# jeong0982/gkr

Measured on AMD Instinct MI355X. Metric: BN254-Fr sumcheck field-ops/sec @ 2^20 vars, higher is better.
Workload: dtype u32x8

## Files before the change

### gkr_amd/csrc/capi_internal.h

```cpp
#pragma once
#include <hip/hip_runtime.h>
#include <sched.h>
#include <stdio.h>
#include <stdlib.h>
#include <string.h>

#include <algorithm>
#include <chrono>
#include <condition_variable>
#include <map>
#include <memory>
#include <mutex>
#include <string>
#include <thread>
#include <vector>

#include "../../include/gkr_amd.h"
#include "fr64.h"
#include "host_cpus.h"
#include "hostpool.h"
#include "kernels.h"
#include "options.h"
#include "gate_seg.h"
#include "keccak.h"
// ... 63 lines not shown
    static const bool adx = !gkr::process_switch("GKR_NO_ADX") && gkr::gkr_adx_available();
    if (!adx) return gkr::h64::mimc7_multi_hash(arr, n, cts, nullptr);
    gkr::h64::F out;
    gkr::gkr_adx_multi_hash(reinterpret_cast<const uint64_t(*)[4]>(arr), n, reinterpret_cast<const uint64_t(*)[4]>(cts), out.l);
    return out;
}

constexpr int kHashChunkMax = 16;
constexpr int kMaxLayerK = GKR_MAX_K_NEXT, kMaxLayerKi = GKR_MAX_K_I, kMaxDenseK = GKR_MAX_K_NEXT_DEVICE_TRANSCRIPT;
inline void ifma_hash_chunk(const uint64_t (*vec)[3][4], const uint32_t* ln, int count, uint64_t (*out)[4]) {
    if (count > 8)
        gkr::gkr_ifma_multi_hash16(vec, ln, 3, out);
    else
        gkr::gkr_ifma_multi_hash8(vec, ln, 3, out);
}
inline int hash_chunk_size(int tables, int threads, int help_share = 0) {
    const long long forced = gkr::opt(gkr::OPT_hash_chunk);
    if (forced == 8 || forced == 16) return (int)forced;
    if (help_share > 1 && tables <= 3 * help_share) return 1;
    return tables >= 32 * threads ? 16 : 8;
}

inline hipError_t device_malloc(void** p, size_t bytes) { return hipMalloc(p, bytes); }
inline hipError_t device_free(void* p) { return hipFree(p); }

inline int default_host_threads() {
    if (const int v = gkr::process_int("GKR_HOST_THREADS", 0); v >= 1) return v;
    int cpus = usable_cpus();
    int local = 1;
    if (const int ranks = gkr::process_int("LOCAL_WORLD_SIZE", 1); ranks > 0) local = ranks;
    const int share = cpus / local;
    int t = share >= 6 ? share - 2 : (share >= 3 ? share - 1 : share);
    if (t < 1) t = 1;
    if (t > 64) t = 64;
    return t;
}

inline Fr to_dev(const gkr_fr& x) {
    Fr f;
    memcpy(&f, &x, 32);
    return f;
}

inline gkr_fr to_abi(const Fr& x) {
    gkr_fr f;
    memcpy(&f, &x, 32);
    return f;
}

inline bool all_canonical(const gkr_fr* v, size_t n) {
    for (size_t i = 0; i < n; ++i)
        if (!gkr::fr_is_canonical(to_dev(v[i]))) return false;
    return true;
}


}
using namespace gkr_host;


struct GateLists {
    uint32_t *offsets = nullptr, *cursor = nullptr, *list = nullptr;
    uint32_t* plan = nullptr;
    gkr::GatePlanCounts plan_counts{};
    gkr::GateSegs segs;
    bool ready = false;
    void release() {
        if (offsets) (void)hipFree(offsets);
        if (cursor) (void)hipFree(cursor);
        if (list) (void)hipFree(list);
        if (plan) (void)hipFree(plan);
        if (segs.words) (void)hipFree(segs.words);
        offsets = cursor = list = plan = nullptr;
        plan_counts = gkr::GatePlanCounts{};
        segs = gkr::GateSegs();
        ready = false;
    }
};
struct PreparedCircuit {
    uint64_t h1 = 0, h2 = 0;
    std::vector<uint32_t> k;
    std::vector<uint8_t*> gt;
    std::vector<uint32_t*> l, r;
    std::vector<GateLists> lists;
    std::vector<unsigned char> retained;
    void release() {
        for (auto p : gt) (void)hipFree(p);
        for (auto p : l) (void)hipFree(p);
        for (auto p : r) (void)hipFree(p);
        for (auto& g : lists) g.release();
        gt.clear();
        l.clear();
        r.clear();
        lists.clear();
    }
};

struct ProveCrew;

struct AsyncWorker {
    std::thread th;
    std::mutex mu;
    std::condition_variable cv;
    std::function<void()> task;
    bool busy = false, stop = false;
    void loop() {
        std::unique_lock<std::mutex> g(mu);
        for (;;) {
            cv.wait(g, [this] { return stop || (busy && task); });
            if (stop) return;
            std::function<void()> t = std::move(task);
            task = nullptr;
            g.unlock();
            t();
            g.lock();
            busy = false;
            cv.notify_all();
        }
    }
    void run(std::function<void()> fn) {
        std::unique_lock<std::mutex> g(mu);
        if (!th.joinable()) th = std::thread([this] { loop(); });
        cv.wait(g, [this] { return !busy; });
        task = std::move(fn);
        busy = true;
        cv.notify_all();
    }
    void wait() {
        std::unique_lock<std::mutex> g(mu);
        cv.wait(g, [this] { return !busy; });
    }
    ~AsyncWorker() {
        {
            std::unique_lock<std::mutex> g(mu);
            cv.wait(g, [this] { return !busy; });
            stop = true;
            cv.notify_all();
        }
        if (th.joinable()) th.join();
    }
};

struct gkr_ctx {
    int device = 0;
    std::vector<int> devices;
    int host_threads = 0;
    gkr::Options options = gkr::Options::from_environment();
    std::vector<std::unique_ptr<PreparedCircuit>> circuits;
    hipStream_t stream = nullptr;
    hipStream_t aux = nullptr;
    hipStream_t late = nullptr;
    hipStream_t chain = nullptr;
    std::vector<hipEvent_t> aux_events;
    Fr* d_cts = nullptr;
    int transcript = GKR_TRANSCRIPT_HOST;
    std::string err;
    int profile = 0;
    std::map<std::string, ProfileRow> prof;
    std::vector<PendingEvent> pending;
    std::vector<hipEvent_t> event_pool;
    char name[256] = {0};
    uint32_t ticket = 0;
    std::unique_ptr<gkr::SpinPool> pool;
    std::unique_ptr<gkr::SpinPool> solo_pool;
    std::unique_ptr<AsyncWorker> copier;
    std::unique_ptr<AsyncWorker> liner;
    void* mle_arrivals_zeroed = nullptr;
    void* arrivals_zeroed = nullptr;
    void* gate_arrive_zeroed = nullptr;
    bool crew_member = false;
    int help_share = 0;
    int rounds_ahead = 0;
    std::unique_ptr<ProveCrew, void (*)(ProveCrew*)> crew{nullptr, nullptr};
    std::map<std::string, std::pair<void*, size_t>> ws;
    std::map<std::string, std::pair<void*, size_t>> pinned;

    hipError_t workspace(const char* slot, size_t bytes, void** out) {
        auto& e = ws[slot];
        if (e.second < bytes) {
            if (e.first) (void)device_free(e.first);
            e.first = nullptr;
            e.second = 0;
            hipError_t rc = device_malloc(&e.first, bytes);
            if (rc != hipSuccess) return rc;
            e.second = bytes;
        }
        *out = e.first;
        return hipSuccess;
    }
    hipError_t pinned_host(const char* slot, size_t bytes, void** out) {
        auto& e = pinned[slot];
        if (e.second < bytes) {
            if (e.first) (void)hipHostFree(e.first);
            e.first = nullptr;
            e.second = 0;
            hipError_t rc = hipHostMalloc(&e.first, bytes, hipHostMallocCoherent | hipHostMallocMapped);
            if (rc != hipSuccess) return rc;
            memset(e.first, 0, bytes);
            e.second = bytes;
        }
        *out = e.first;
        return hipSuccess;
    }
    void release_buffers() {
        for (auto& c : circuits) c->release();
        circuits.clear();
        for (auto& kv : ws)
            if (kv.second.first) (void)device_free(kv.second.first);
        ws.clear();
        for (auto& kv : pinned)
            if (kv.second.first) (void)hipHostFree(kv.second.first);
        pinned.clear();
    }
    int threads() const { return host_threads > 0 ? host_threads : default_host_threads(); }
    gkr::SpinPool* host_pool() {
        if (crew_member) {
            if (!solo_pool) solo_pool.reset(new gkr::SpinPool(0));
            return solo_pool.get();
        }
        if (!pool) pool.reset(new gkr::SpinPool(threads() - 1));
        return pool.get();
    }
    hipError_t late_stream(hipStream_t* out) {
        if (!late) {
            const hipError_t rc = hipStreamCreateWithFlags(&late, hipStreamNonBlocking);
            if (rc != hipSuccess) return rc;
        }
        *out = late;
        return hipSuccess;
    }
    hipError_t chain_stream(hipStream_t* out) {
        if (!chain) {
            hipError_t rc = hipStreamCreateWithFlags(&chain, hipStreamNonBlocking);
            if (rc != hipSuccess) return rc;
        }
        *out = chain;
        return hipSuccess;
    }
    hipError_t aux_stream(int events) {
        if (!aux) {
            hipError_t rc = hipStreamCreateWithFlags(&aux, hipStreamNonBlocking);
            if (rc != hipSuccess) return rc;
        }
        while ((int)aux_events.size() < events) {
            hipEvent_t e;
            hipError_t rc = hipEventCreateWithFlags(&e, hipEventDisableTiming);
            if (rc != hipSuccess) return rc;
            aux_events.push_back(e);
        }
        return hipSuccess;
    }

    int fail(int status, const std::string& what) {
        err = what;
        return status;
    }
    int hip_fail(hipError_t e, const char* what) {
        err = std::string(what) + ": " + hipGetErrorString(e);
        return GKR_ERR_HIP;
    }
    hipEvent_t get_event() {
        if (!event_pool.empty()) {
            hipEvent_t e = event_pool.back();
            event_pool.pop_back();
            return e;
        }
        hipEvent_t e;
        (void)hipEventCreate(&e);
        return e;
    }
    void add_host_sample(const char* name, double ms) {
        ProfileRow& r = prof[name];
        r.launches += 1;
        r.total_ms += ms;
        if (r.samples.size() < kMaxSamples) r.samples.emplace_back((float)ms, 0.0);
    }
    void drain_events() {
        for (auto& p : pending) {
            (void)hipEventSynchronize(p.stop);
            float ms = 0.f;
            (void)hipEventElapsedTime(&ms, p.start, p.stop);
            ProfileRow& r = prof[p.name];
            r.launches += 1;
            r.total_ms += ms;
            r.bytes += p.bytes;
            if (r.samples.size() < kMaxSamples) r.samples.emplace_back(ms, p.bytes);
            event_pool.push_back(p.start);
            event_pool.push_back(p.stop);
        }
        pending.clear();
    }
};

struct ProveCrew {
    struct Member {
        gkr_ctx* ctx = nullptr;
        std::thread th;
        std::vector<int> items;
    };
    std::vector<std::unique_ptr<Member>> members;
    std::mutex mu;
    std::condition_variable cv_start, cv_done;
    uint64_t generation = 0;
    bool stop = false;
    int active = 0;
    int finished = 0;
    gkr_prove_item* items = nullptr;
    const std::vector<std::vector<int>>* units = nullptr;
    int32_t busy = 0;
    double t_call_us = 0;
};

struct Timed {
    gkr_ctx* c;
    PendingEvent ev;
    bool on;
    hipStream_t st;
    Timed(gkr_ctx* ctx, const char* name, double bytes, hipStream_t stream = nullptr, bool minor = false)
        : c(ctx), on(ctx->profile == 1 || (ctx->profile == 2 && !minor)), st(stream ? stream : ctx->stream) {
        if (on) {
            ev.start = c->get_event();
            ev.stop = c->get_event();
            ev.name = name;
            ev.bytes = bytes;
            (void)hipEventRecord(ev.start, st);
        }
    }
    ~Timed() {
        if (on) {
            (void)hipEventRecord(ev.stop, st);
            c->pending.push_back(ev);
        }
    }
};

#define GKR_ENTER(ctx)                                        \
    HIP_TRY(ctx, hipSetDevice((ctx)->device));                \
    gkr::OptionScope gkr_option_scope_(&(ctx)->options)

#define HIP_TRY(ctx, expr)                                   \
    do {                                                     \
        hipError_t _e = (expr);                              \
        if (_e != hipSuccess) return (ctx)->hip_fail(_e, #expr); \
    } while (0)


namespace gkr_host {


template <typename T>
struct DevBuf {
    T* p = nullptr;
    ~DevBuf() {
        if (p) (void)hipFree(p);
    }
    hipError_t alloc(size_t count) { return hipMalloc(reinterpret_cast<void**>(&p), count * sizeof(T)); }
};

template <typename Run>
int run_on_upload(gkr_ctx* ctx, const gkr_fr* host, size_t count, Run run) {
    GKR_ENTER(ctx);
    DevBuf<Fr> d;
    HIP_TRY(ctx, d.alloc(count));
    HIP_TRY(ctx, hipMemcpyAsync(d.p, host, count * sizeof(Fr), hipMemcpyHostToDevice, ctx->stream));
    return run(d.p);
}
template <typename Run>
int run_on_tables(gkr_ctx* ctx, const gkr_fr* tables, size_t count, Run run) {
    if (!all_canonical(tables, count)) return ctx->fail(GKR_ERR_NON_CANONICAL, "table entry >= r");
    return run_on_upload(ctx, tables, count, run);
}

struct ThreadTimeAccount {
    double own_pieces_us = 0, helped_us = 0, spin_us = 0;
};
inline thread_local ThreadTimeAccount t_account;
struct HostAccountTotals {
    std::atomic<uint64_t> own_ns{0}, helped_ns{0}, spin_ns{0}, rest_ns{0}, lent_ns{0}, lent_idle_ns{0}, calls{0}, wake_ns{0};
    std::atomic<uint64_t> pieces{0}, piece_ns{0}, piece_pass_ns{0}, lanes[17] = {};
    std::atomic<bool> on{false};
};
inline HostAccountTotals& host_account_totals() {
    static HostAccountTotals t;
    return t;
}
inline bool accounting_on() { return host_account_totals().on.load(std::memory_order_relaxed); }
inline void account_piece(int transcripts, double pass_us, double total_us) {
    HostAccountTotals& t = host_account_totals();
    t.pieces.fetch_add(1, std::memory_order_relaxed);
    t.piece_ns.fetch_add((uint64_t)(total_us * 1e3), std::memory_order_relaxed);
    t.piece_pass_ns.fetch_add((uint64_t)(pass_us * 1e3), std::memory_order_relaxed);
    t.lanes[transcripts < 1 ? 1 : (transcripts > 16 ? 16 : transcripts)].fetch_add(1, std::memory_order_relaxed);
}
inline double now_us_dbg() { return std::chrono::duration<double, std::micro>(std::chrono::steady_clock::now().time_since_epoch()).count(); }

inline bool help_enabled() {
    static const bool on = !gkr::process_switch("GKR_NO_HELP");
    return on;
}
static void run_pieces(gkr::SpinPool* pool, const std::function<bool()>* work, bool several, int priority = 0) {
    auto run = [&] {
        if (pool)
            pool->run_now(work);
        else
            while ((*work)()) {
// ... 216 lines not shown
```

### gkr_amd/csrc/capi_mle_passes.hip

```cpp
#include "capi_internal.h"

namespace gkr_host {

void host_pass_scalar(const uint64_t* sums, size_t sums_row_words, int count, int J, const uint32_t* final_len,
                             uint64_t (*c0)[16][4], uint64_t (*c1)[16][4], uint64_t (*r)[16][4], uint32_t (*len)[16],
                             uint64_t* weights, size_t w_row_words) {
    using gkr::h64::F;
    const F* cts = host_mimc_constants64();
    const F one_m = gkr::h64::to_mont(F{{1, 0, 0, 0}});
    for (int k = 0; k < count; ++k) {
        F S[gkr::kMleMaxSub], rm[gkr::kMlePassMaxRounds];
        memcpy(S, sums + (size_t)k * sums_row_words, sizeof(F) << J);
        for (int t = 0; t < J; ++t) {
            const int half = 1 << (J - t - 1);
            F lo = S[0], hi = S[half];
            for (int b = 1; b < half; ++b) {
                lo = gkr::h64::add(lo, S[b]);
                hi = gkr::h64::add(hi, S[half + b]);
            }
            const F d = gkr::h64::sub(hi, lo);
            const uint32_t ln = (final_len && t == J - 1) ? final_len[k] : (gkr::h64::is_zero(d) ? 1u : 2u);
            const F vec[2] = {d, lo};
            const F rc = host_multi_hash(vec + (2 - ln), (int)ln, cts);
            memcpy(c0[t][k], &lo, 32);
            memcpy(c1[t][k], &d, 32);
            memcpy(r[t][k], &rc, 32);
            len[t][k] = ln;
            rm[t] = gkr::h64::to_mont(rc);
            for (int b = 0; b < half; ++b) S[b] = gkr::h64::add(S[b], gkr::h64::mont_mul(gkr::h64::sub(S[half + b], S[b]), rm[t]));
        }
        if (!weights) continue;
        F* w = reinterpret_cast<F*>(weights + (size_t)k * w_row_words);
        F tmp[gkr::kMleMaxSub];
        tmp[0] = one_m;
        int cur = 1;
        for (int t = 0; t < J; ++t) {
            const F nr = gkr::h64::sub(one_m, rm[t]);
            for (int b = cur; b-- > 0;) {
                tmp[2 * b + 1] = gkr::h64::mont_mul(tmp[b], rm[t]);
                tmp[2 * b] = gkr::h64::mont_mul(tmp[b], nr);
            }
            cur <<= 1;
        }
        memcpy(w, tmp, sizeof(F) << J);
    }
}

struct MlePassTables {
    const Fr* input = nullptr;
    size_t in_stride = 0;
    Fr* work = nullptr;
    size_t work_len = 0;
    gkr::MleSubPartial* partials = nullptr;
    unsigned char* plans = nullptr;
    Fr* h_w = nullptr;
    Fr *h_w2 = nullptr, *d_w2 = nullptr;
    gkr::MleHostRecSub* h_rec = nullptr;
    gkr::MleHostRecSub* rec = nullptr;
    uint32_t* arrivals = nullptr;
    Fr* h_tail = nullptr;
};
static int mle_pass_tables(gkr_ctx* ctx, const std::string& prefix, const Fr* input, size_t len, size_t work_len, int batch, MlePassTables& T) {
    T.input = input;
    T.in_stride = len;
    T.work_len = work_len;
    WS(ctx, (prefix + ".work").c_str(), Fr, (size_t)batch * (work_len ? work_len : 1), T.work);
    WS(ctx, (prefix + ".partials").c_str(), gkr::MleSubPartial, (size_t)batch * gkr::kMaxBlocksPerTable, T.partials);
    WS(ctx, (prefix + ".plans").c_str(), unsigned char, (size_t)batch * gkr::mle_fold_plan_bytes(), T.plans);
    HIP_TRY(ctx, ctx->pinned_host((prefix + ".rec").c_str(), sizeof(gkr::MleHostRecSub) * batch, reinterpret_cast<void**>(&T.h_rec)));
    HIP_TRY(ctx, ctx->pinned_host((prefix + ".w").c_str(), sizeof(Fr) * gkr::kMleMaxSub * batch, reinterpret_cast<void**>(&T.h_w)));
    T.rec = T.h_rec;
    return GKR_OK;
}

constexpr double kFusedPublishBytes = 64.0 * 1024 * 1024;
constexpr uint32_t kFusedPublishBlocks = 256;
constexpr size_t kArrivalCounters = 4096;
static int mle_arrival_counters(gkr_ctx* ctx, size_t len, MlePassTables& T) {
    if (gkr::opt(gkr::OPT_no_fused_reduce) != 0 || (double)len * 32.0 > kFusedPublishBytes) return GKR_OK;
    WS(ctx, "mlep.arrivals", uint32_t, kArrivalCounters, T.arrivals);
    if (ctx->mle_arrivals_zeroed != T.arrivals) {
        HIP_TRY(ctx, hipMemsetAsync(T.arrivals, 0, sizeof(uint32_t) * kArrivalCounters, ctx->stream));
        ctx->mle_arrivals_zeroed = T.arrivals;
    }
    return GKR_OK;
}
static bool fused_publish(const MlePassTables& T, int b0, int nb, uint32_t nblk, double bytes_read, uint32_t ticket, int jout, gkr::MlePublish& pub) {
    if (!T.arrivals || (size_t)(b0 + nb) > kArrivalCounters || bytes_read > kFusedPublishBytes || (uint64_t)nblk * nb > kFusedPublishBlocks || nblk > 128u)
        return false;
    pub.rec = T.rec + b0;
    pub.arrivals = T.arrivals + b0;
    pub.ticket = ticket;
    pub.jout = (uint32_t)jout;
    return true;
}

constexpr uint32_t kMleTailLog2 = 7;
struct MlePassPolicy {
    const char* row = nullptr;
    int plan_event = -1;
    Fr* export_tail = nullptr;
    int blocks_jout = 0;
    uint32_t src_planes = 1;
};
static uint32_t pass0_blocks(size_t len, int jout, int nb, const MlePassPolicy& P) {
    uint32_t nblk = gkr::mle_pass_blocks((uint32_t)len, (uint32_t)(P.blocks_jout > 0 ? P.blocks_jout : jout), nb);
    if (P.blocks_jout > 0 && len / nblk < 256u) nblk = (uint32_t)(len / 256u);
    return nblk;
}
static void queue_sub_reduce(gkr_ctx* ctx, const MlePassTables& T, int b0, int nb, uint32_t nblk, int jout, uint32_t ticket, hipStream_t st) {
    Timed t(ctx, "mle_sub_reduce", 0.0, st, true);
    gkr::launch_mle_sub_reduce(T.partials + (size_t)b0 * gkr::kMaxBlocksPerTable, nblk, (uint32_t)jout, nb, T.rec + b0, ticket, st);
}
static void queue_pass0(gkr_ctx* ctx, const MlePassTables& T, int b0, int nb, int jout, uint32_t ticket, hipStream_t st, const MlePassPolicy& P) {
    const size_t len = T.in_stride;
    const Fr* src = T.input + (size_t)b0 * len;
    const double bytes = (double)nb * len * 32.0;
    if (len <= gkr::kSmallPassEntries) {
        Timed t(ctx, "mle_pass_small", bytes, st, true);
        gkr::launch_mle_multifold_small(0, src, len, nullptr, 0, (uint32_t)len, (uint32_t)jout, nb, T.h_w + (size_t)b0 * gkr::kMleMaxSub, T.rec + b0, ticket, st);
        return;
    }
    const uint32_t nblk = pass0_blocks(len, jout, nb, P);
    gkr::MlePublish pub;
    const bool fused = fused_publish(T, b0, nb, nblk, bytes, ticket, jout, pub);
    {
        Timed t(ctx, P.row, bytes, st, fused);
        gkr::launch_mle_sub_sums(src, len, (uint32_t)len, nb, nblk, T.partials + (size_t)b0 * gkr::kMaxBlocksPerTable, st, fused ? &pub : nullptr);
    }
    if (!fused) queue_sub_reduce(ctx, T, b0, nb, nblk, jout, ticket, st);
}
static void queue_fold(gkr_ctx* ctx, const MlePassTables& T, int b0, int nb, bool from_input, int m_src, int jin, int jout, uint32_t ticket,
                       hipStream_t st, const MlePassPolicy& P) {
    const size_t src_len = (size_t)1 << m_src, S = src_len >> jin;
    const Fr* src = from_input ? T.input + (size_t)b0 * T.in_stride : T.work + (size_t)b0 * T.work_len;
    const size_t src_stride = from_input ? T.in_stride : T.work_len;
    Fr* dst = T.work + (size_t)b0 * T.work_len;
    const Fr* w = T.h_w + (size_t)b0 * gkr::kMleMaxSub;
    const double bytes = (double)nb * ((double)src_len * P.src_planes + (double)S) * 32.0;
    if (S <= gkr::kSmallPassEntries) {
        Timed t(ctx, "mle_pass_small", bytes, st, true);
        gkr::launch_mle_multifold_small(jin, src, src_stride, dst, T.work_len, (uint32_t)S, (uint32_t)jout, nb, w, T.rec + b0, ticket, st, P.export_tail,
                                        1u << kMleTailLog2, P.src_planes, (uint32_t)src_len);
        return;
    }
    const uint32_t nblk = gkr::mle_multifold_blocks((uint32_t)S, (uint32_t)jout, nb);
    unsigned char* plan = T.plans + (size_t)b0 * gkr::mle_fold_plan_bytes();
    if (gkr::mle_multifold_uses_mfma((uint32_t)S, nblk)) {
        if (P.plan_event < 0) {
            gkr::launch_mle_fold_plan(jin, w, plan, nb, st);
        } else {
            {
                Timed t(ctx, "mle_fold_plan", 0.0, ctx->aux, true);
                gkr::launch_mle_fold_plan(jin, w, plan, nb, ctx->aux);
            }
            (void)hipEventRecord(ctx->aux_events[P.plan_event], ctx->aux);
            (void)hipStreamWaitEvent(st, ctx->aux_events[P.plan_event], 0);
        }
    }
    gkr::MlePublish pub;
    const bool fused = fused_publish(T, b0, nb, nblk, (double)nb * (double)src_len * 32.0, ticket, jout, pub);
    {
        Timed t(ctx, P.row, bytes, st, fused);
        gkr::launch_mle_multifold(jin, src, src_stride, dst, T.work_len, (uint32_t)S, nb, nblk, w, plan, T.partials + (size_t)b0 * gkr::kMaxBlocksPerTable, st,
                                  fused ? &pub : nullptr);
    }
    if (!fused) queue_sub_reduce(ctx, T, b0, nb, nblk, jout, ticket, st);
}

struct MleSchedule {
    int jmax = 0, j_first = 0;
    int n_dev = 0;
    int groups = 0, depth = 0;
    int bound[kMaxGroups + 1];
    uint32_t chunk[kMaxGroups];
    bool tail_on = false;
    bool two_level = false;
};
static MleSchedule mle_schedule(int n, int batch, int hash_threads, bool is_tail, const gkr::Options& o) {
    MleSchedule sc;
    const double len = (double)((size_t)1 << n);
    const int jcap = o.v[gkr::OPT_no_mfma_fold] ? 3 : gkr::kMlePassMaxRounds;
    const int jwant = o.v[gkr::OPT_rounds_per_pass] > 0 ? (int)o.v[gkr::OPT_rounds_per_pass] : jcap;
    sc.jmax = jwant > jcap ? jcap : jwant;
    sc.j_first = mle_pass_rounds(n, n, sc.jmax);
    sc.two_level = !is_tail && mle_two_level_first_fold(n, o);
    const long long dp = o.v[gkr::OPT_device_hash_percent];
    const int dev_percent = dp < 0 ? 0 : (dp > 90 ? 90 : (int)dp);
    if (dev_percent > 0 && !is_tail && batch >= 64 && sc.j_first >= 1) {
        sc.n_dev = (int)((long long)batch * dev_percent / 100) & ~7;
        if (batch - sc.n_dev < 16) sc.n_dev = (batch - 16) & ~7;
        if (sc.n_dev < 8) sc.n_dev = 0;
    }
    const int host_batch = batch - sc.n_dev;
    const double batch_bytes = (double)host_batch * len * 32.0;
    int want_groups = (int)(batch_bytes / (4.0 * 1024 * 1024 * 1024));
    want_groups = want_groups < 4 ? 4 : (want_groups > 8 ? (batch_bytes > 96.0 * 1024 * 1024 * 1024 ? 16 : 8) : want_groups);
    const bool small_tables = n <= 17 && host_batch >= 256;
    if (small_tables) want_groups = 16;
    if (hash_threads <= 3 && host_batch >= 256 && want_groups < 16) want_groups = 16;
    int group_size = host_batch >= 128 ? (host_batch + want_groups - 1) / want_groups : (host_batch >= 16 ? (host_batch + 1) / 2 : host_batch);
    if (sc.n_dev && hash_threads <= 3 && host_batch >= 256) group_size = 64;
    if (o.v[gkr::OPT_group_size] > 0) group_size = (int)o.v[gkr::OPT_group_size];
    sc.groups = (host_batch + group_size - 1) / group_size;
    if (sc.groups > kMaxGroups) sc.groups = kMaxGroups;
    const long long forced = o.v[gkr::OPT_hash_chunk];
    for (int g = 0; g <= sc.groups; ++g) sc.bound[g] = sc.n_dev + (int)((long long)host_batch * g / sc.groups);
    for (int g = 0; g < sc.groups; ++g) {
        const int nb = sc.bound[g + 1] - sc.bound[g], per = (nb + hash_threads - 1) / hash_threads;
        sc.chunk[g] = forced == 8 || forced == 16 ? (uint32_t)forced : (nb >= 32 * hash_threads ? 16u : (uint32_t)(per <= 8 ? 8 : (per <= 16 ? per : 16)));
    }
    sc.depth = o.v[gkr::OPT_pass_queue_depth] > 0 ? (int)o.v[gkr::OPT_pass_queue_depth] : (small_tables ? 4 : 2);
    sc.tail_on = o.v[gkr::OPT_host_tail_log2] >= 0 && sc.n_dev == 0 && batch <= (o.v[gkr::OPT_host_tail_max_batch] > 0 ? o.v[gkr::OPT_host_tail_max_batch] : 8);
    return sc;
}

namespace {
struct PassGroup : GroupHandoff {
    int m = 0;
    int j = 0;
    int round0 = 0;
    int pass = 0, index = 0;
    hipStream_t chain = nullptr;
    bool on_host = false;
    bool mid = false, planes = false;
};
struct MlePassClock {
    const bool on = gkr::debug_timing();
    const std::chrono::steady_clock::time_point t0 = std::chrono::steady_clock::now();
    double a = 0, b = 0, c = 0, d = 0, e = 0;
    std::atomic<uint64_t> busy_ns{0};
    double us() const { return std::chrono::duration<double, std::micro>(std::chrono::steady_clock::now() - t0).count(); }
    void report(int threads) const {
        if (!on) return;
        fprintf(stderr,
                "[gkr timing] setup %.0f us, first launches %.0f, loop %.0f, end_session %.0f, sync %.0f, drain %.0f; hashing %.0f us "
                "over %d threads = %.0f%% of the loop\n",
                a, b - a, c - b, d - c, e - d, us() - e, busy_ns.load() * 1e-3, threads, busy_ns.load() * 1e-3 / ((c - b) * threads) * 100.0);
    }
};

struct MlePassRun {
    gkr_ctx* ctx;
    const int n, batch;
    const MleTailArgs* tail;
    gkr_fr* out_coeffs;
    uint32_t* out_len;
    gkr_fr* out_r;
    MleSchedule sc;
    MlePassTables T;
    hipStream_t s = nullptr, late = nullptr, chain = nullptr;
    std::vector<PassGroup> grp;
    std::vector<uint32_t> dep_last;
    int next_first = 0;
    gkr_fr *stage_c = nullptr, *stage_r = nullptr;
    uint32_t* stage_len = nullptr;
    MlePassClock clock;

    int rounds_for(int m) const { return mle_pass_rounds(m, n, sc.jmax); }
    void advance(PassGroup& G, int jin) {
        G.m -= jin;
        G.round0 += jin;
        G.j = rounds_for(G.m);
        G.ticket = ++ctx->ticket;
    }
    void launch_first(PassGroup& G) {
        G.ticket = ++ctx->ticket;
        MlePassPolicy P;
        P.row = G.chain ? "mle_sub_sums_dev" : "mle_sub_sums";
        if (two_level(G)) P.blocks_jout = kMleTwoLevelRounds;
        queue_pass0(ctx, T, G.b0, G.nb, G.j, G.ticket, G.chain ? G.chain : s, P);
    }
    void launch_next_first() {
        if (next_first < sc.groups) launch_first(grp[next_first++]);
    }
    void launch_fold(PassGroup& G, int jin) {
        const int m_src = G.m;
        const bool from_input = m_src == n;
        hipStream_t st = G.chain ? G.chain : ((!from_input && m_src <= 16) ? late : s);
        advance(G, jin);
        MlePassPolicy P;
        P.row = G.chain ? "mle_multifold_dev" : (st == s ? "mle_multifold" : "mle_multifold_late");
        if (!gkr::opt(gkr::OPT_plan_main) && st == s && sc.groups != 1) P.plan_event = G.index;
        G.on_host = sc.tail_on && !G.chain && G.m <= (int)kMleTailLog2 && G.m - G.j > 0;
        if (G.on_host) P.export_tail = T.h_tail + ((size_t)G.b0 << kMleTailLog2);
        if (G.planes) P.src_planes = gkr::kMleFold2Planes;
        G.planes = false;
        queue_fold(ctx, T, G.b0, G.nb, from_input, m_src, jin, G.j, G.ticket, st, P);
    }
    bool two_level(const PassGroup& G) const { return sc.two_level && !G.chain; }
    bool side_launches() const { return !gkr::opt(gkr::OPT_plan_main) && sc.groups != 1; }
    void launch_fine_sums(PassGroup& G) {
        const int J = G.j;
        G.mid = true;
        G.round0 += J;
        G.ticket = ++ctx->ticket;
        hipStream_t side = side_launches() ? ctx->aux : s;
        MlePassPolicy P0;
        P0.blocks_jout = kMleTwoLevelRounds;
        const uint32_t nblk0 = pass0_blocks(T.in_stride, J, G.nb, P0);
        const Fr* w = T.h_w + (size_t)G.b0 * gkr::kMleMaxSub;
        Timed t(ctx, "mle_fold_plan", 0.0, side, true);
        gkr::launch_mle_fine_sums(T.partials + (size_t)G.b0 * gkr::kMaxBlocksPerTable, nblk0, w, G.nb, T.rec + G.b0, G.ticket, side);
        gkr::launch_mle_fold_plan(J, w, T.plans + (size_t)G.b0 * gkr::mle_fold_plan_bytes(), G.nb, side, side == s ? 0u : 256u);
    }
    void launch_fold2(PassGroup& G) {
        const bool side = side_launches();
        {
            Timed t(ctx, "mle_fold_plan", 0.0, side ? ctx->aux : s, true);
            gkr::launch_mle_copy_weights(T.h_w2 + (size_t)G.b0 * gkr::kMleMaxSub, T.d_w2 + (size_t)G.b0 * gkr::kMleMaxSub, G.nb, side ? ctx->aux : s);
        }
        if (side) {
            (void)hipEventRecord(ctx->aux_events[G.index], ctx->aux);
            (void)hipStreamWaitEvent(s, ctx->aux_events[G.index], 0);
        }
        const uint32_t S = 1u << (n - gkr::kMlePassMaxRounds), npart = gkr::mle_multifold2_partials(S);
        G.mid = false;
        G.planes = true;
        G.on_host = false;
        G.m = n - kMleTwoLevelRounds;
        G.round0 += G.j;
        G.j = gkr::kMlePassMaxRounds;
        G.ticket = ++ctx->ticket;
        {
            Timed t(ctx, "mle_multifold", (double)G.nb * ((double)T.in_stride + (double)(gkr::kMleFold2Planes * (S >> gkr::kMlePassMaxRounds))) * 32.0, s);
            gkr::launch_mle_multifold2(T.input + (size_t)G.b0 * T.in_stride, T.in_stride, T.work + (size_t)G.b0 * T.work_len, T.work_len, S, G.nb,
                                       T.plans + (size_t)G.b0 * gkr::mle_fold_plan_bytes(), T.d_w2 + (size_t)G.b0 * gkr::kMleMaxSub,
                                       T.partials + (size_t)G.b0 * gkr::kMaxBlocksPerTable, s);
        }
        queue_sub_reduce(ctx, T, G.b0, G.nb, npart, G.j, G.ticket, s);
    }
    void host_fold(PassGroup& G, int jin) {
        using gkr::h64::F;
        advance(G, jin);
        const size_t S = (size_t)1 << G.m, nsub = (size_t)1 << G.j, sub = S >> G.j;
        for (int b = G.b0; b < G.b0 + G.nb; ++b) {
            F* tab = reinterpret_cast<F*>(T.h_tail + ((size_t)b << kMleTailLog2));
            const F* w = reinterpret_cast<const F*>(T.h_w + (size_t)b * gkr::kMleMaxSub);
            for (size_t i = 0; i < S; ++i) {
                gkr::h64::Wide acc = gkr::h64::wide_zero();
                for (size_t t = 0; t < ((size_t)1 << jin); ++t) gkr::h64::wide_mac(acc, tab[t * S + i], w[t]);
                tab[i] = gkr::h64::wide_reduce(acc);
            }
            F* sums = reinterpret_cast<F*>(T.h_rec[b].sums);
            for (size_t a = 0; a < nsub; ++a) {
                F v = tab[a * sub];
                for (size_t i = 1; i < sub; ++i) v = gkr::h64::add(v, tab[a * sub + i]);
                sums[a] = v;
            }
            __atomic_store_n(&T.h_rec[b].seq, G.ticket, __ATOMIC_RELEASE);
        }
    }
    void process_chunk(const PassGroup& G, int b_first, int count) {
        static const bool scalar_book = gkr::process_switch("GKR_HOST_PASS_SCALAR");
        const int J = G.j, n_out = tail ? tail->n_total : n, r_off = tail ? tail->round_offset : 0;
        uint64_t c0[gkr::kMlePassMaxRounds][16][4], c1[gkr::kMlePassMaxRounds][16][4], r[gkr::kMlePassMaxRounds][16][4];
        uint32_t ln[gkr::kMlePassMaxRounds][16], final_len[16];
        const bool final_pass = G.round0 + J == n;
        for (int i = 0; i < count; ++i) {
            if (G.round0 == 0) dep_last[b_first + i] = tail && tail->dep_last ? tail->dep_last[b_first + i] : T.h_rec[b_first + i].dep;
            final_len[i] = dep_last[b_first + i] ? 2u : 1u;
        }
        static_assert(sizeof(gkr::MleHostRecSub) % 8 == 0, "hand-off records are addressed in 64-bit words");
        const uint64_t* sums = reinterpret_cast<const uint64_t*>(T.h_rec[b_first].sums);
        uint64_t* weights = G.m - J > 0 ? reinterpret_cast<uint64_t*>((G.mid ? T.h_w2 : T.h_w) + (size_t)b_first * gkr::kMleMaxSub) : nullptr;
        (host_ifma_ready() && count >= 3 && !scalar_book ? gkr::gkr_ifma_pass : host_pass_scalar)(
            sums, sizeof(gkr::MleHostRecSub) / 8, count, J, final_pass ? final_len : nullptr, c0, c1, r, ln, weights, 4 * gkr::kMleMaxSub);
        for (int i = 0; i < count; ++i)
            for (int t = 0; t < J; ++t)
                write_round_output(out_coeffs, out_len, out_r, (size_t)(b_first + i) * n_out + r_off + G.round0 + t, c0[t][i], c1[t][i], ln[t][i], r[t][i]);
    }
    bool try_work() {
        for (;;) {
            int best = -1;
            uint32_t best_gen = 0;
            for (int g = 0; g < sc.groups; ++g)
                if (const uint32_t gen = grp[g].open_generation(); gen && (best < 0 || gen < best_gen)) best = g, best_gen = gen;
            if (best < 0) return false;
            PassGroup& G = grp[best];
            uint32_t first, take;
            if (!G.try_claim(sc.chunk[best], &first, &take)) continue;
            const double t_in = clock.on ? clock.us() : 0.0;
            process_chunk(G, G.b0 + (int)first, (int)take);
            G.finish(take);
            if (clock.on) clock.busy_ns.fetch_add((uint64_t)((clock.us() - t_in) * 1e3), std::memory_order_relaxed);
            return true;
        }
    }
    int queue_device_chain() {
        const int n_dev = sc.n_dev;
        HIP_TRY(ctx, ctx->chain_stream(&chain));
        uint32_t* dep_dev = nullptr;
        WS(ctx, "mlep.dev_dep", uint32_t, (size_t)n_dev, dep_dev);
        HIP_TRY(ctx, ctx->pinned_host("mlep.stage_c", sizeof(gkr_fr) * 2 * (size_t)n_dev * n, reinterpret_cast<void**>(&stage_c)));
        HIP_TRY(ctx, ctx->pinned_host("mlep.stage_r", sizeof(gkr_fr) * (size_t)n_dev * n, reinterpret_cast<void**>(&stage_r)));
        HIP_TRY(ctx, ctx->pinned_host("mlep.stage_len", sizeof(uint32_t) * (size_t)n_dev * n, reinterpret_cast<void**>(&stage_len)));
        PassGroup dev;
        dev.nb = n_dev;
        dev.m = n;
        dev.j = sc.j_first;
        dev.index = sc.groups;
        dev.chain = chain;
        launch_first(dev);
        for (bool first = true;; first = false) {
            const int J = dev.j;
            {
                Timed t(ctx, "mle_pass_hash_dev", 0.0, chain);
                gkr::launch_mle_pass_hash_lanes(T.rec, (uint32_t)n_dev, (uint32_t)J, (uint32_t)dev.round0, (uint32_t)n, dev.round0 + J == n, first, ctx->d_cts,
                                                dep_dev, dev.m - J > 0 ? T.h_w : nullptr, reinterpret_cast<Fr*>(stage_c), stage_len,
                                                reinterpret_cast<Fr*>(stage_r), chain);
            }
            if (dev.m - J <= 0) return GKR_OK;
            launch_fold(dev, J);
        }
    }
    bool step(PassGroup& G, int& active) {
        if (G.state == 0 && G.records_landed(T.h_rec)) {
            G.open((uint32_t)++G.pass);
            return true;
        }
        if (G.state != 1 || !G.all_done()) return false;
        if (G.m - G.j > 0) {
            const bool first_fold = G.m == n;
            if (first_fold && two_level(G) && !G.mid) {
                launch_fine_sums(G);
                G.state = 0;
                return true;
            }
            if (first_fold && two_level(G))
                launch_fold2(G);
            else if (G.on_host)
                host_fold(G, G.j);
            else
                launch_fold(G, G.j);
            G.state = 0;
            if (first_fold) launch_next_first();
        } else {
            G.state = 2;
            --active;
            launch_next_first();
        }
        return true;
    }
    int loop() {
        int rc = GKR_OK, active = sc.groups;
        HandoffWatch watch{ctx, s, "pass"};
        while (active > 0 && rc == GKR_OK) {
            bool progress = false;
            for (int g = 0; g < next_first; ++g) progress |= step(grp[g], active);
            if (progress)
                rc = watch.progressed();
            else if (!try_work())
                rc = watch.idled();
        }
        return rc;
    }
};
}

int run_mle_batch_passes(gkr_ctx* ctx, const Fr* d_tables, int n, int batch, gkr_fr* out_coeffs, uint32_t* out_len, gkr_fr* out_r,
                         const MleTailArgs* tail) {
    MlePassRun R{ctx, n, batch, tail, out_coeffs, out_len, out_r};
    const size_t len = (size_t)1 << n;
    hipStream_t s = R.s = R.late = ctx->stream;
    gkr::SpinPool* pool = ctx->host_pool();
    const gkr::Options* o = gkr::current_options();
    const MleSchedule& sc = R.sc = mle_schedule(n, batch, pool->workers() + 1, tail != nullptr, o ? *o : gkr::default_options());
    if (int rc = mle_pass_tables(ctx, "mlep", d_tables, len, len >> sc.j_first, batch, R.T)) return rc;
    if (int rc = mle_arrival_counters(ctx, len, R.T)) return rc;
    if (sc.two_level) {
        HIP_TRY(ctx, ctx->pinned_host("mlep.w2", sizeof(Fr) * gkr::kMleMaxSub * batch, reinterpret_cast<void**>(&R.T.h_w2)));
        WS(ctx, "mlep.d_w2", Fr, (size_t)batch * gkr::kMleMaxSub, R.T.d_w2);
    }
    HIP_TRY(ctx, ctx->aux_stream(sc.groups));
    if (sc.tail_on) HIP_TRY(ctx, ctx->pinned_host("mlep.tail", sizeof(Fr) * ((size_t)batch << kMleTailLog2), reinterpret_cast<void**>(&R.T.h_tail)));
    if (!gkr::opt(gkr::OPT_no_late_stream) && sc.groups > 1) HIP_TRY(ctx, ctx->late_stream(&R.late));
    R.dep_last = std::vector<uint32_t>(batch, 0);
    R.grp = std::vector<PassGroup>(sc.groups);
    for (int g = 0; g < sc.groups; ++g) {
        PassGroup& G = R.grp[g];
        G.index = g;
        G.b0 = sc.bound[g];
        G.nb = sc.bound[g + 1] - sc.bound[g];
        G.m = n;
        G.j = sc.j_first;
    }
    const std::function<bool()> try_work = [&R] { return R.try_work(); };
    R.clock.a = R.clock.us();
    gkr::SpinPool::Session session(pool, &try_work);
    R.launch_next_first();
    if (sc.n_dev)
        if (int rc = R.queue_device_chain()) return rc;
    while (R.next_first < sc.groups && R.next_first < sc.depth) R.launch_next_first();
    R.clock.b = R.clock.us();
    const int rc = R.loop();
    R.clock.c = R.clock.us();
    session.close();
    if (rc) {
        (void)hipStreamSynchronize(s);
        if (R.late != s) (void)hipStreamSynchronize(R.late);
        if (R.chain) (void)hipStreamSynchronize(R.chain);
        ctx->mle_arrivals_zeroed = nullptr;
        return rc;
    }
    R.clock.d = R.clock.us();
    HIP_TRY(ctx, hipGetLastError());
    HIP_TRY(ctx, hipStreamSynchronize(s));
    if (R.late != s) HIP_TRY(ctx, hipStreamSynchronize(R.late));
    if (sc.n_dev) {
        HIP_TRY(ctx, hipStreamSynchronize(R.chain));
        memcpy(out_coeffs, R.stage_c, sizeof(gkr_fr) * 2 * (size_t)sc.n_dev * n);
        memcpy(out_r, R.stage_r, sizeof(gkr_fr) * (size_t)sc.n_dev * n);
        memcpy(out_len, R.stage_len, sizeof(uint32_t) * (size_t)sc.n_dev * n);
    }
    R.clock.e = R.clock.us();
    if (ctx->pending.size() > 8192) ctx->drain_events();
    R.clock.report(pool->workers() + 1);
    return GKR_OK;
}

namespace {
struct MleShardRun {
    gkr_ctx* ctx;
    const gkr_exchange_dev* exchange;
    const int n, batch;
    gkr_fr* out_coeffs;
    uint32_t* out_len;
    gkr_fr* out_r;
    MlePassTables T;
    uint32_t* h_fail = nullptr;
    std::vector<uint32_t> dep_last;
    gkr::SpinPool* pool = nullptr;
    int rc = GKR_OK;
    uint32_t exchanges = 0;

    long long* limbs() const { return reinterpret_cast<long long*>(exchange->d_limbs); }
    void hook_failed(int arc) {
        if (arc && !rc) rc = ctx->fail(GKR_ERR_INVALID, "the device sum-over-ranks hook failed (status " + std::to_string(arc) + ")");
    }
    bool some_rank_failed() const { return __atomic_load_n(h_fail, __ATOMIC_ACQUIRE) != 0; }
    void exchange_sums(int J, uint32_t ticket) {
        hipStream_t s = ctx->stream;
        Timed t(ctx, "exchange", 0.0);
        gkr::launch_mle_xwiden(T.rec, (uint32_t)J, (uint32_t)batch, rc ? 1u : 0u, limbs(), s);
        const int arc = exchange->fn(exchange->user, (size_t)batch * (((size_t)1 << J) + 2) * 8, static_cast<void*>(s));
        gkr::launch_mle_xnarrow(limbs(), (uint32_t)J, (uint32_t)batch, T.h_rec, ticket, h_fail, s);
        ++exchanges;
        hook_failed(arc);
    }
    void gather_tail(const Fr* rest, size_t stride, int m, int lp, int shard, Fr* d_tail) {
        hipStream_t s = ctx->stream;
        Timed t(ctx, "exchange", 0.0);
        gkr::launch_mle_gather_widen(rest, stride, (uint32_t)m, (uint32_t)lp, (uint32_t)shard, rc ? 1u : 0u, (uint32_t)batch, limbs(), s);
        const int arc = exchange->fn(exchange->user, ((size_t)batch << (m + lp)) * 8 + 8, static_cast<void*>(s));
        gkr::launch_mle_gather_narrow(limbs(), (uint32_t)(m + lp), (uint32_t)batch, d_tail, h_fail, s);
        ++exchanges;
        hook_failed(arc);
    }
    void rounds_chunk(int first, int J, int round0) {
        const int count = batch - first < 16 ? batch - first : 16;
        uint64_t c0[gkr::kMlePassMaxRounds][16][4], c1[gkr::kMlePassMaxRounds][16][4], r[gkr::kMlePassMaxRounds][16][4];
        uint32_t ln[gkr::kMlePassMaxRounds][16];
        (host_ifma_ready() && count >= 3 ? gkr::gkr_ifma_pass : host_pass_scalar)(
            reinterpret_cast<const uint64_t*>(T.h_rec[first].sums), sizeof(gkr::MleHostRecSub) / 8, count, J, nullptr, c0, c1, r, ln,
            reinterpret_cast<uint64_t*>(T.h_w + (size_t)first * gkr::kMleMaxSub), 4 * gkr::kMleMaxSub);
        for (int i = 0; i < count; ++i) {
            if (round0 == 0) dep_last[first + i] = T.h_rec[first + i].dep;
            for (int t = 0; t < J; ++t)
                write_round_output(out_coeffs, out_len, out_r, (size_t)(first + i) * n + round0 + t, c0[t][i], c1[t][i], ln[t][i], r[t][i]);
        }
    }
    void host_rounds(int J, int round0) {
        std::atomic<int> next{0};
        const std::function<bool()> work_fn = [&]() -> bool {
            const int first = next.fetch_add(16, std::memory_order_relaxed);
            if (first < batch) rounds_chunk(first, J, round0);
            return first < batch;
        };
        gkr::SpinPool::Session session(pool, nullptr);
        run_pieces(pool, &work_fn, batch > 16);
    }
    void pass(bool pass0, bool from_input, int m_src, int jin, int J, int round0) {
        const uint32_t ticket = ++ctx->ticket;
        if (!rc) {
            MlePassPolicy P;
            P.row = pass0 ? "mle_sub_sums" : "mle_multifold";
            if (pass0)
                queue_pass0(ctx, T, 0, batch, J, ticket, ctx->stream, P);
            else
                queue_fold(ctx, T, 0, batch, from_input, m_src, jin, J, ticket, ctx->stream, P);
            if (hipError_t le = hipGetLastError(); le != hipSuccess) rc = ctx->hip_fail(le, "launch of a sumcheck pass");
        }
        exchange_sums(J, ticket);
        if (!rc) rc = wait_records(ctx, T.h_rec, batch, ticket);
        if (!rc && some_rank_failed()) rc = ctx->fail(GKR_ERR_HIP, "another rank failed during the sumcheck");
        if (!rc) host_rounds(J, round0);
    }
};
}

}

extern "C" {

size_t gkr_exchange_limbs_mle(int n, int log2_shards, int batch) {
    if (n < 2 || log2_shards < 0 || log2_shards > 16 || n - log2_shards < 1 || n - log2_shards > GKR_MAX_MLE_N || batch < 1) return 0;
    const int nl = n - log2_shards, t = nl < kMleShardTailLog2 ? nl : kMleShardTailLog2;
    const size_t per_pass = (size_t)batch * (gkr::kMleMaxSub + 2) * 8, gather = ((size_t)batch << (t + log2_shards)) * 8 + 8;
    return per_pass > gather ? per_pass : gather;
}

int gkr_sumcheck_mle_sharded_dev(gkr_ctx* ctx, const void* d_shards, int n, int log2_shards, int shard, int batch,
                                 const gkr_exchange_dev* exchange, gkr_fr* out_coeffs, uint32_t* out_len, gkr_fr* out_r,
                                 uint32_t* out_exchanges) {
    if (!ctx) return GKR_ERR_INVALID;
    if (!d_shards || !exchange || !exchange->fn || !exchange->d_limbs || !out_coeffs || !out_len || !out_r || batch < 1 || batch > 65535)
        return ctx->fail(GKR_ERR_INVALID, "null pointer or batch out of range [1, 65535]");
    const int lp = log2_shards, nl = n - lp;
    if (lp < 0 || lp > 16 || shard < 0 || shard >= (1 << lp)) return ctx->fail(GKR_ERR_INVALID, "shard must be in [0, 2^log2_shards), log2_shards in [0, 16]");
    if (n < 2 || nl < 1 || nl > GKR_MAX_MLE_N) return ctx->fail(GKR_ERR_INVALID, "n >= 2 and 1 <= n - log2_shards <= GKR_MAX_MLE_N needed");
    if (ctx->transcript != GKR_TRANSCRIPT_HOST) return ctx->fail(GKR_ERR_INVALID, "a sumcheck split over ranks needs the host transcript");
    if (exchange->capacity < gkr_exchange_limbs_mle(n, lp, batch)) return ctx->fail(GKR_ERR_INVALID, "the exchange buffer is smaller than gkr_exchange_limbs_mle(n, log2_shards, batch) int64");
    GKR_ENTER(ctx);
    hipStream_t s = ctx->stream;
    const size_t len = (size_t)1 << nl;
    const int t_stop = nl < kMleShardTailLog2 ? nl : kMleShardTailLog2;
    const int jmax = gkr::opt(gkr::OPT_no_mfma_fold) ? 3 : gkr::kMlePassMaxRounds;
    auto rounds_for = [&](int m) {
        int j = mle_pass_rounds(m, nl, jmax);
        if (m - j < t_stop) j = m - t_stop;
        return j;
    };
    MleShardRun R{ctx, exchange, n, batch, out_coeffs, out_len, out_r};
    MlePassTables& T = R.T;
    Fr* d_tail = nullptr;
    const int j_first = nl > t_stop ? rounds_for(nl) : 0;
    if (int rc = mle_pass_tables(ctx, "mlex", static_cast<const Fr*>(d_shards), len, j_first ? len >> j_first : 1, batch, T)) return rc;
    WS(ctx, "mlex.tail", Fr, (size_t)batch << (t_stop + lp), d_tail);
    WS(ctx, "mlex.drec", gkr::MleHostRecSub, (size_t)batch, T.rec);
    HIP_TRY(ctx, ctx->pinned_host("mlex.fail", 64, reinterpret_cast<void**>(&R.h_fail)));
    *R.h_fail = 0;
    R.dep_last = std::vector<uint32_t>(batch, 0);
    R.pool = batch >= 32 ? ctx->host_pool() : nullptr;
    int m = nl, round0 = 0, jin = 0;
    while (m - jin > t_stop) {
        m -= jin;
        const int J = rounds_for(m);
        R.pass(jin == 0, round0 == jin, m + jin, jin, J, round0);
        round0 += J;
        jin = J;
    }
    m -= jin;
    const bool folded = jin && !R.rc;
    if (folded) {
        MlePassPolicy P;
        P.row = "mle_multifold";
        queue_fold(ctx, T, 0, batch, round0 == jin, m + jin, jin, 1, ++ctx->ticket, s, P);
        if (hipError_t le = hipGetLastError(); le != hipSuccess) R.rc = ctx->hip_fail(le, "launch of the last rank-local fold");
    }
    R.gather_tail(folded ? T.work : T.input, folded ? T.work_len : len, m, lp, shard, d_tail);
    if (out_exchanges) *out_exchanges = R.exchanges;
    {
        const hipError_t se = hipStreamSynchronize(s);
        if (se != hipSuccess && !R.rc) R.rc = ctx->hip_fail(se, "hipStreamSynchronize after the gather");
    }
    if (!R.rc && R.some_rank_failed()) R.rc = ctx->fail(GKR_ERR_HIP, "another rank failed during the sumcheck");
    if (R.rc) return R.rc;
    ctx->drain_events();
    MleTailArgs tail;
    tail.n_total = n;
    tail.round_offset = round0;
    tail.dep_last = round0 ? R.dep_last.data() : nullptr;
    return run_mle_batch_passes(ctx, d_tail, m + lp, batch, out_coeffs, out_len, out_r, &tail);
}

}
```

### gkr_amd/csrc/gkr_capi.hip

```cpp
#include "capi_internal.h"


extern "C" {

const char* gkr_strerror(int status) {
    switch (status) {
        case GKR_OK: return "ok";
        case GKR_ERR_INVALID: return "invalid argument";
        case GKR_ERR_NON_CANONICAL: return "field element is not canonical (>= r)";
        case GKR_ERR_NO_DEVICE: return "no gfx950 device available";
        case GKR_ERR_HIP: return "HIP runtime error";
        case GKR_ERR_NOMEM: return "out of memory";
        case GKR_ERR_DEGENERATE: return "degenerate sumcheck (v == 0)";
        case GKR_ERR_UNSUPPORTED: return "R1CS shape the reference's compiler does not support";
        default: return "unknown status";
    }
}

const char* gkr_version(void) { return "gkr_amd 0.1 (gfx950)"; }

int gkr_ctx_create(int device_id, gkr_ctx** out) {
    if (!out) return GKR_ERR_INVALID;
    *out = nullptr;
    int count = 0;
    if (hipGetDeviceCount(&count) != hipSuccess || count <= 0) return GKR_ERR_NO_DEVICE;
    if (device_id < 0 || device_id >= count) return GKR_ERR_INVALID;
    struct RestoreDevice {
        int prev = -1;
        RestoreDevice() {
            if (hipGetDevice(&prev) != hipSuccess) prev = -1;
        }
        ~RestoreDevice() {
            if (prev >= 0) (void)hipSetDevice(prev);
        }
    } restore_device;
    if (hipSetDevice(device_id) != hipSuccess) return GKR_ERR_HIP;
    gkr_ctx* c = new gkr_ctx();
    c->device = device_id;
    hipDeviceProp_t prop;
    if (hipGetDeviceProperties(&prop, device_id) == hipSuccess)
        snprintf(c->name, sizeof c->name, "%s (%s, %d CUs)", prop.name, prop.gcnArchName, prop.multiProcessorCount);
    if (hipStreamCreateWithFlags(&c->stream, hipStreamNonBlocking) != hipSuccess) {
        delete c;
        return GKR_ERR_HIP;
    }
    if (hipMalloc(reinterpret_cast<void**>(&c->d_cts), sizeof(Fr) * gkr::kMimcRounds) != hipSuccess ||
        hipMemcpy(c->d_cts, host_mimc_constants(), sizeof(Fr) * gkr::kMimcRounds, hipMemcpyHostToDevice) != hipSuccess) {
        gkr_ctx_destroy(c);
        return GKR_ERR_HIP;
    }
    *out = c;
    return GKR_OK;
}

int gkr_ctx_create_multi(const int* device_ids, int n_devices, gkr_ctx** out) {
    if (!out) return GKR_ERR_INVALID;
    *out = nullptr;
    if (!device_ids || n_devices < 1 || n_devices > 64) return GKR_ERR_INVALID;
    int count = 0;
    if (hipGetDeviceCount(&count) != hipSuccess || count <= 0) return GKR_ERR_NO_DEVICE;
    for (int i = 0; i < n_devices; ++i)
        if (device_ids[i] < 0 || device_ids[i] >= count) return GKR_ERR_INVALID;
    gkr_ctx* c = nullptr;
    const int rc = gkr_ctx_create(device_ids[0], &c);
    if (rc) return rc;
    c->devices.assign(device_ids, device_ids + n_devices);
    *out = c;
    return GKR_OK;
}

int gkr_ctx_device_count(const gkr_ctx* ctx) { return ctx ? (ctx->devices.empty() ? 1 : (int)ctx->devices.size()) : 0; }

void gkr_ctx_destroy(gkr_ctx* ctx) {
    if (!ctx) return;
    ctx->crew.reset();
    (void)hipSetDevice(ctx->device);
    if (ctx->stream) (void)hipStreamSynchronize(ctx->stream);
    if (ctx->aux) (void)hipStreamSynchronize(ctx->aux);
    if (ctx->late) (void)hipStreamSynchronize(ctx->late);
    ctx->drain_events();
    ctx->drain_events();
    for (hipEvent_t e : ctx->event_pool) (void)hipEventDestroy(e);
    ctx->release_buffers();
    if (ctx->d_cts) (void)hipFree(ctx->d_cts);
    for (hipEvent_t e : ctx->aux_events) (void)hipEventDestroy(e);
    if (ctx->aux) (void)hipStreamDestroy(ctx->aux);
    if (ctx->late) (void)hipStreamDestroy(ctx->late);
    if (ctx->chain) (void)hipStreamDestroy(ctx->chain);
    if (ctx->stream) (void)hipStreamDestroy(ctx->stream);
    delete ctx;
}

const char* gkr_last_error(const gkr_ctx* ctx) { return ctx ? ctx->err.c_str() : "null context"; }

int gkr_ctx_set_transcript(gkr_ctx* ctx, int mode) {
    if (!ctx || (mode != GKR_TRANSCRIPT_DEVICE && mode != GKR_TRANSCRIPT_HOST)) return GKR_ERR_INVALID;
    ctx->transcript = mode;
    return GKR_OK;
}

int gkr_option_count(void) { return (int)gkr::OPT_COUNT; }
const char* gkr_option_name(int index) { return index >= 0 && index < (int)gkr::OPT_COUNT ? gkr::option_table()[index].name : nullptr; }
const char* gkr_option_doc(int index) { return index >= 0 && index < (int)gkr::OPT_COUNT ? gkr::option_table()[index].doc : nullptr; }
const char* gkr_option_env(int index) { return index >= 0 && index < (int)gkr::OPT_COUNT ? gkr::option_table()[index].env : nullptr; }

int gkr_ctx_get_option(const gkr_ctx* ctx, const char* name, long long* value) {
    const int i = gkr::option_index(name);
    if (!ctx || !value || i < 0) return GKR_ERR_INVALID;
    *value = ctx->options.v[i];
    return GKR_OK;
}

int gkr_ctx_set_option(gkr_ctx* ctx, const char* name, long long value) {
    if (!ctx) return GKR_ERR_INVALID;
    const int i = gkr::option_index(name);
    if (i < 0) return ctx->fail(GKR_ERR_INVALID, std::string("unknown option: ") + (name ? name : "(null)"));
    if (ctx->crew_member) return ctx->fail(GKR_ERR_INVALID, "options of a context that is proving are not changed");
    if (ctx->options.v[i] == value) return GKR_OK;
    int prev_device = -1;
    if (hipGetDevice(&prev_device) != hipSuccess) prev_device = -1;
    auto drop_cache = [](gkr_ctx* c) {
        if (hipSetDevice(c->device) != hipSuccess) return;
        if (c->stream) (void)hipStreamSynchronize(c->stream);
        if (c->aux) (void)hipStreamSynchronize(c->aux);
        for (auto& pc : c->circuits) pc->release();
        c->circuits.clear();
    };
    drop_cache(ctx);
    ctx->options.v[i] = value;
    if (ctx->crew)
        for (size_t m = 1; m < ctx->crew->members.size(); ++m) {
            gkr_ctx* child = ctx->crew->members[m]->ctx;
            if (!child) continue;
            drop_cache(child);
            child->options = ctx->options;
        }
    if (prev_device >= 0) (void)hipSetDevice(prev_device);
    return GKR_OK;
}

int gkr_ctx_set_host_threads(gkr_ctx* ctx, int threads) {
    if (!ctx || threads < 0 || threads > 256) return GKR_ERR_INVALID;
    if (threads != ctx->host_threads) {
        ctx->pool.reset();
        ctx->host_threads = threads;
    }
    return GKR_OK;
}

long gkr_host_help_while(const volatile int32_t* busy) {
    if (!busy) return 0;
    long pieces = 0;
    unsigned idle = 0;
    const bool account = accounting_on();
    const double t0 = account ? now_us_dbg() : 0.0;
    double lent_us = 0;
    while (__atomic_load_n(busy, __ATOMIC_ACQUIRE) != 0) {
        const double th = account ? now_us_dbg() : 0.0;
        if (help_enabled() && gkr::HelpBoard::instance().help()) {
            if (account) lent_us += now_us_dbg() - th;
            ++pieces;
            idle = 0;
            continue;
        }
        GKR_CPU_RELAX();
        if (++idle > 4096) {
            std::this_thread::yield();
            idle = 0;
        }
    }
    if (account) {
        HostAccountTotals& tot = host_account_totals();
        const double all = now_us_dbg() - t0;
        tot.lent_ns.fetch_add((uint64_t)(lent_us * 1e3), std::memory_order_relaxed);
        tot.lent_idle_ns.fetch_add((uint64_t)((all > lent_us ? all - lent_us : 0) * 1e3), std::memory_order_relaxed);
    }
    return pieces;
}

int gkr_host_accounting(int enable) {
    HostAccountTotals& tot = host_account_totals();
    if (enable) {
        tot.own_ns = 0;
        tot.helped_ns = 0;
        tot.spin_ns = 0;
        tot.rest_ns = 0;
        tot.lent_ns = 0;
        tot.lent_idle_ns = 0;
        tot.calls = 0;
        tot.wake_ns = 0;
        tot.pieces = 0;
        tot.piece_ns = 0;
        tot.piece_pass_ns = 0;
        for (auto& l : tot.lanes) l = 0;
    }
    tot.on.store(enable != 0, std::memory_order_relaxed);
    return GKR_OK;
}

int gkr_host_accounting_read(double* out_us, size_t count) {
    if (!out_us || count < 7) return GKR_ERR_INVALID;
    if (count >= 8) out_us[7] = host_account_totals().wake_ns.load() * 1e-3;
    const HostAccountTotals& tot = host_account_totals();
    out_us[0] = tot.own_ns.load() * 1e-3;
    out_us[1] = tot.helped_ns.load() * 1e-3;
    out_us[2] = tot.spin_ns.load() * 1e-3;
    out_us[3] = tot.rest_ns.load() * 1e-3;
    out_us[4] = tot.lent_ns.load() * 1e-3;
    out_us[5] = tot.lent_idle_ns.load() * 1e-3;
    out_us[6] = (double)tot.calls.load();
    if (count >= 28) {
        out_us[8] = (double)tot.pieces.load();
        out_us[9] = tot.piece_ns.load() * 1e-3;
        out_us[10] = tot.piece_pass_ns.load() * 1e-3;
        for (int n = 1; n <= 16; ++n) out_us[10 + n] = (double)tot.lanes[n].load();
        out_us[27] = 0.0;
    }
    return GKR_OK;
}

int gkr_ctx_device_name(const gkr_ctx* ctx, char* buf, size_t len) {
    if (!ctx || !buf || !len) return GKR_ERR_INVALID;
    snprintf(buf, len, "%s", ctx->name);
    return GKR_OK;
}

int gkr_ctx_profile(gkr_ctx* ctx, int enable) {
    if (!ctx) return GKR_ERR_INVALID;
    ctx->profile = enable < 0 ? 0 : (enable > 2 ? 2 : enable);
    return GKR_OK;
}

int gkr_ctx_profile_get(gkr_ctx* ctx, const char* kernel, uint64_t* launches, double* total_ms, double* bytes) {
    if (!ctx || !kernel) return GKR_ERR_INVALID;
    ctx->drain_events();
    auto it = ctx->prof.find(kernel);
    ProfileRow r = it == ctx->prof.end() ? ProfileRow() : it->second;
    if (launches) *launches = r.launches;
// ... 509 lines not shown
```

### gkr_amd/csrc/kernels.h

```cpp
#pragma once
#include <hip/hip_runtime.h>
#include <stddef.h>
#include <stdint.h>

#include "fr32.h"

namespace gkr {

constexpr uint32_t kMaxBlocksPerTable = 2048;
constexpr uint32_t kMaxLayerBlocks = 2048;

struct MlePartial {
    Acc<9> lo, hi;
    uint32_t dep, pad;
};

struct LayerBatch {
    uint32_t batch;
    uint32_t pstride;
    size_t tstride, wstride;
};
inline LayerBatch single_layer() { return LayerBatch{1u, 0u, 0, 0}; }

struct LayerPartial {
    Acc<9> c0, g1, c2;
    uint32_t pad;
};

struct MleHostRec {
    Fr c0, c1;
    uint32_t dep, seq;
    uint32_t pad[14];
};
struct LayerHostRec {
    Fr c0, g1, c2;
    uint32_t seq;
    uint32_t pad[7];
};
static_assert(sizeof(MleHostRec) == 128 && sizeof(LayerHostRec) == 128, "hand-off records are one 128-byte line");

constexpr int kProdMaxJ = 3;
constexpr int kProdRecValues = 72;
struct ProdPassRec {
    Fr v[kProdRecValues];
    uint32_t seq;
    uint32_t pad[7];
};
static_assert(sizeof(ProdPassRec) == kProdRecValues * 32 + 32, "product-pass record layout");
constexpr uint32_t kProdTile = 8, kProdTileWide = 32;
inline uint32_t prod_pass_tile(uint32_t S) { return S >= 1024u ? kProdTileWide : kProdTile; }
inline uint32_t prod_pass_blocks(uint32_t S) { return S <= kProdTile ? 1u : S / prod_pass_tile(S); }
inline uint32_t prod_pass_max_blocks(uint32_t k) {
    uint32_t m = 1;
    for (uint32_t l = 0; l < k; ++l) m = prod_pass_blocks(1u << l) > m ? prod_pass_blocks(1u << l) : m;
    return m;
}
inline size_t prod_pass_scratch_values(uint32_t k) { return ((size_t)prod_pass_max_blocks(k) + 64u) * kProdRecValues; }
constexpr uint32_t kProdFuseBlocks = 64;
constexpr uint32_t kProdFoldMinM = 17;
size_t prod_fold_plan_bytes();
void launch_prod_pass(Fr* W, Fr* X, Fr* Y, uint32_t m_in, uint32_t jp, const Fr* weights, uint32_t J, Fr* partials, uint32_t wstride,
                      ProdPassRec* rec, uint32_t ticket, uint32_t batch, hipStream_t s, uint32_t* arrivals = nullptr, void* fold_plans = nullptr,
                      Fr* tail = nullptr, uint32_t tail_stride = 0);
void launch_prod_c_setup(const Fr* Wb, uint32_t jp, const Fr* weights, const Fr* A, const Fr* M, Fr* X, Fr* Y, uint32_t k, uint32_t wstride,
                         uint32_t batch, hipStream_t s);

constexpr uint32_t kSmallFoldQuarter = 2048;
void launch_mle_fold_sum_small(const Fr* src, size_t src_stride, Fr* dst, size_t dst_stride, uint32_t q, uint32_t batch,
                               const FixedMul* rtab, MleHostRec* host_rec, uint32_t ticket, hipStream_t s);
void launch_mle_round_reduce(const MlePartial* partials, uint32_t nblk, uint32_t batch, MleHostRec* host_rec,
                             uint32_t ticket, hipStream_t s);

struct MleSubPartial {
    Acc<9> sum;
    uint32_t dep, pad[2];
};
constexpr int kMlePassMaxRounds = 5;
constexpr int kMleMaxSub = 1 << kMlePassMaxRounds;
struct MleHostRecSub {
    Fr sums[kMleMaxSub];
    uint32_t dep, seq;
    uint32_t pad[14];
};
static_assert(sizeof(MleHostRecSub) == 1088, "hand-off record layout");
struct MlePublish {
    MleHostRecSub* rec = nullptr;
    uint32_t* arrivals = nullptr;
    uint32_t ticket = 0, jout = 0;
};
constexpr uint32_t kSmallPassEntries = 512;
uint32_t mle_pass_blocks(uint32_t items, uint32_t jout, uint32_t batch);
uint32_t mle_multifold_blocks(uint32_t S, uint32_t jout, uint32_t batch);
bool mle_multifold_uses_mfma(uint32_t S, uint32_t nblk);
constexpr int kMlePass0Stream = 3;
constexpr uint64_t kMlePass0DeepMinPartials = 2u * 12u * 256u * 4u;
void launch_mle_sub_sums(const Fr* tables, size_t stride, uint32_t len, uint32_t batch, uint32_t nblk, MleSubPartial* partials,
                         hipStream_t s, const MlePublish* publish = nullptr);
void launch_mle_sub_reduce(const MleSubPartial* partials, uint32_t nblk, uint32_t jout, uint32_t batch, MleHostRecSub* host_rec,
                           uint32_t ticket, hipStream_t s);
size_t mle_fold_plan_bytes();
void launch_mle_fold_plan(int jin, const Fr* weights, void* plans, uint32_t batch, hipStream_t s, uint32_t threads = 0);
void launch_mle_multifold(int jin, const Fr* src, size_t src_stride, Fr* dst, size_t dst_stride, uint32_t S, uint32_t batch,
                          uint32_t nblk, const Fr* weights, const void* plans, MleSubPartial* partials, hipStream_t s,
                          const MlePublish* publish = nullptr);
void launch_mle_pass_hash_lanes(const MleHostRecSub* rec, uint32_t count, uint32_t J, uint32_t round0, uint32_t n_out, bool final_pass,
                                bool first_pass, const Fr* cts, uint32_t* dep_last, Fr* weights, Fr* out_coeffs, uint32_t* out_len, Fr* out_r,
                                hipStream_t s);
void launch_mle_multifold_small(int jin, const Fr* src, size_t src_stride, Fr* dst, size_t dst_stride, uint32_t S, uint32_t jout,
                                uint32_t batch, const Fr* weights, MleHostRecSub* host_rec, uint32_t ticket, hipStream_t s, Fr* tail = nullptr, uint32_t tail_stride = 0,
                                uint32_t planes = 1, uint32_t plane_stride = 0);
constexpr uint32_t kMleFold2Planes = 8;
uint32_t mle_multifold2_partials(uint32_t S);
uint32_t mle_multifold2_tiles(uint32_t S);
void launch_mle_fine_sums(const MleSubPartial* partials, uint32_t nblk, const Fr* weights, uint32_t batch, MleHostRecSub* host_rec, uint32_t ticket,
                          hipStream_t s);
void launch_mle_copy_weights(const Fr* src, Fr* dst, uint32_t batch, hipStream_t s);
void launch_mle_multifold2(const Fr* src, size_t src_stride, Fr* dst, size_t dst_stride, uint32_t S, uint32_t batch, const void* plans, const Fr* w2,
                           MleSubPartial* partials, hipStream_t s);
void launch_layer_round_reduce(const LayerPartial* partials, uint32_t nblk, LayerHostRec* host_rec, uint32_t ticket,
                               LayerBatch lb, hipStream_t s);
void launch_fold_small(Fr* W, uint32_t hw, const FixedMul* rtab, LayerBatch lb, hipStream_t s);
struct GateSpan {
    uint64_t base, count;
};
uint32_t gate_lists_lds_blocks(uint64_t gates, uint32_t k);
size_t gate_lists_lds_scratch_words(uint64_t gates, uint32_t k);
inline size_t gate_list_words(uint64_t gates) { return 2 * (size_t)gates + 1; }
struct GateSegs {
    uint32_t shift = 0;
    uint32_t runs = 0;
    uint32_t run_base = 0;
    uint32_t bound = 0;
    uint32_t half_bound = 0;
    uint32_t groups = 0;
    uint32_t nb = 0;
    uint64_t packed_half = 0;
    uint32_t* words = nullptr;
    uint2* items() const { return reinterpret_cast<uint2*>(words); }
    uint32_t* order() const { return words + 2 * (size_t)bound; }
    uint32_t* bucket_begin() const { return order() + bound; }
    uint32_t* group_len() const { return bucket_begin() + 2 * (size_t)nb + 2; }
    uint32_t* group_off() const { return group_len() + 2 * (size_t)groups; }
    uint32_t* packed() const { return group_off() + 2 * (size_t)groups + 2; }
};
uint32_t gate_seg_shift(GateSpan span, uint32_t k_i, uint32_t k);
size_t gate_segs_words(GateSpan span, uint32_t k_i, uint32_t k);
size_t gate_segs_scratch_words(GateSpan span, uint32_t k_i, uint32_t k);
size_t gate_seg_partial_elems(GateSpan span, uint32_t k_i, uint32_t k);
void launch_gate_lists(GateSpan span, uint32_t k_i, uint32_t k, const uint8_t* gate_type, const uint32_t* left, const uint32_t* right,
                       uint32_t* counts, uint32_t* offsets, uint32_t* cursor, uint32_t* block_sums, uint32_t* list, uint32_t* bad,
                       uint32_t* lds_scratch, GateSegs* segs, uint32_t* seg_scratch, hipStream_t s);
struct GateSet {
    const uint32_t* offsets;
    const uint32_t* cursor;
    const uint32_t* list;
    const uint32_t* plan;
    const uint8_t* gate_type;
    const uint32_t* left;
    const uint32_t* right;
    uint64_t pad;
};
static_assert(sizeof(GateSet) == 64, "one cache line per proof");
void launch_gate_uv(GateSpan span, uint32_t k_i, uint32_t k, const uint32_t* offsets, const uint32_t* cursor, const uint32_t* list,
                    const Fr* e_hi, const Fr* e_lo_mont, uint32_t kl, const Fr* W, Fr* U, Fr* V, LayerBatch lb, const GateSegs* segs,
                    Fr* partials, hipStream_t s, const GateSet* sets = nullptr);
struct CPhaseFuse {
    const Fr* Wb = nullptr;
    const Fr* weights = nullptr;
    Fr* X = nullptr;
    Fr* Y = nullptr;
    uint32_t jp = 0;
};
bool launch_gate_rows(GateSpan span, uint32_t k_i, uint32_t k, const uint32_t* offsets, const uint32_t* cursor, const uint32_t* list,
                      const Fr* e_hi, const Fr* e_lo_mont, uint32_t kl, const Fr* eq_mont, Fr* A_row, Fr* M_row, LayerBatch lb,
                      const GateSegs* segs, Fr* partials, hipStream_t s, const CPhaseFuse* fuse = nullptr, const GateSet* sets = nullptr);
void launch_fill_table(Fr* table, size_t count, uint64_t seed, hipStream_t s);
void launch_fill_shard(Fr* shard_table, size_t count, uint32_t lp, uint32_t shard, uint64_t seed, hipStream_t s);
void launch_exchange_widen(const Fr* a, const Fr* b, uint32_t each, const uint32_t* flag, uint32_t local_flag, long long* limbs, hipStream_t s);
void launch_exchange_narrow(const long long* limbs, Fr* a, Fr* b, uint32_t each, uint32_t* flag_out, hipStream_t s);
void launch_ubench_copy(const void* in, void* out, size_t bytes, hipStream_t s);
void launch_ubench_read(const void* in, void* out, size_t bytes, hipStream_t s);
void launch_ubench_modmul(Fr* io, uint32_t entries_pow2, uint32_t waves, int reps, hipStream_t s);

uint32_t mle_blocks_per_table(uint32_t items, uint32_t batch);
void launch_mle_sum_first(const Fr* tables, size_t stride, uint32_t h, uint32_t batch, uint32_t nblk,
                          MlePartial* partials, hipStream_t s);
void launch_mle_fold_sum(const Fr* src, size_t src_stride, Fr* dst, size_t dst_stride, uint32_t q, uint32_t batch,
                         uint32_t nblk, const FixedMul* rtab, uint32_t r_stride, MlePartial* partials, hipStream_t s);
void launch_mle_round_hash(const MlePartial* partials, uint32_t nblk, uint32_t round, uint32_t n, uint32_t batch,
                           const Fr* cts, Fr* out_coeffs, uint32_t* out_len, Fr* out_r, FixedMul* rtab,
                           uint32_t* dep_last, hipStream_t s);

constexpr int kProductMaxDegree = 3;
struct ProductPartial {
    Acc<9> s[kProductMaxDegree + 1];
    uint32_t flags, pad[3];
};
void launch_product_first(int degree, const Fr* tables, size_t table_stride, uint32_t h, uint32_t batch, uint32_t nblk,
                          ProductPartial* partials, hipStream_t s);
void launch_product_fold_sum(int degree, const Fr* src, size_t src_stride, Fr* dst, size_t dst_stride, uint32_t q, uint32_t batch,
                             uint32_t nblk, const FixedMul* rtab, uint32_t r_stride, ProductPartial* partials, hipStream_t s);
void launch_product_round(int degree, const ProductPartial* partials, uint32_t nblk, uint32_t round, uint32_t n, uint32_t batch,
                          const Fr* cts, const Fr* work, size_t work_stride, Fr* out_coeffs, uint32_t* out_len, Fr* out_r,
                          FixedMul* rtab, uint32_t* meta, Fr* evals, hipStream_t s);

constexpr int kSopMaxTables = 8, kSopMaxTerms = 8;
struct SopTerms {
    uint32_t n_tables, n_terms, max_degree;
    uint32_t term[kSopMaxTerms];
};
struct SopCoeffs {
    Fr c[kSopMaxTerms];
};
void launch_sop_first(const SopTerms& ts, const Fr* tables, size_t table_stride, uint32_t h, uint32_t batch, uint32_t nblk,
                      ProductPartial* partials, hipStream_t s);
void launch_sop_fold_sum(const SopTerms& ts, const Fr* src, size_t src_stride, Fr* dst, size_t dst_stride, uint32_t q, uint32_t batch,
                         uint32_t nblk, const FixedMul* rtab, uint32_t r_stride, ProductPartial* partials, hipStream_t s);
void launch_sop_round(const SopTerms& ts, const SopCoeffs& cf, const ProductPartial* partials, uint32_t nblk, uint32_t round, uint32_t n,
                      uint32_t batch, const Fr* cts, const Fr* work, size_t work_stride, Fr* out_coeffs, uint32_t* out_len, Fr* out_r,
                      FixedMul* rtab, Fr* evals, hipStream_t s);

struct ZcWeights {
    Fr *hi, *lo;
    uint32_t batch;
    const Fr* hi_table(uint32_t m) const { return hi + (size_t)batch * ((1u << m) - 1u); }
    const Fr* lo_table(uint32_t k) const { return lo + (size_t)batch * ((1u << k) - 1u); }
};
size_t zc_weight_elements(uint32_t n, uint32_t batch);
ZcWeights zc_weights_layout(Fr* base, uint32_t n, uint32_t batch);
void launch_zc_weights(const Fr* points, uint32_t n, uint32_t batch, const ZcWeights& w, hipStream_t s);
void launch_zc_first(const SopTerms& ts, const Fr* tables, size_t table_stride, uint32_t h, uint32_t batch, uint32_t nblk, const ZcWeights& w,
                     uint32_t kh, uint32_t kl, ProductPartial* partials, hipStream_t s);
void launch_zc_fold_sum(const SopTerms& ts, const Fr* src, size_t src_stride, Fr* dst, size_t dst_stride, uint32_t q, uint32_t batch,
                        uint32_t nblk, const FixedMul* rtab, uint32_t r_stride, const ZcWeights& w, uint32_t kh, uint32_t kl,
                        ProductPartial* partials, hipStream_t s);
void launch_zc_round(const SopTerms& ts, const SopCoeffs& cf, const ProductPartial* partials, uint32_t nblk, uint32_t round, uint32_t n,
                     uint32_t batch, const Fr* cts, const Fr* z, Fr* s_slot, const Fr* work, size_t work_stride, Fr* out_coeffs,
                     uint32_t* out_len, Fr* out_r, FixedMul* rtab, Fr* evals, Fr* eq_out, hipStream_t s);

void launch_layer_eval(uint32_t gates, const uint8_t* gate_type, const uint32_t* left, const uint32_t* right,
                       const Fr* prev, Fr* out, uint32_t batch, uint32_t prev_stride, hipStream_t s, const GateSet* sets = nullptr);
void launch_copy_words(const void* src, void* dst, size_t words, hipStream_t s);
void launch_copy_rows(const void* src, size_t src_stride_words, void* dst, size_t dst_stride_words, uint32_t words, uint32_t rows, hipStream_t s);
void launch_eq_table(const Fr* points, uint32_t stride, uint32_t first, uint32_t nvars, Fr* out, bool montgomery, uint32_t batch,
                     hipStream_t s, const CPhaseFuse* wu_job = nullptr, Fr* wu_out = nullptr, uint32_t wstride = 0);
void launch_layer_prologue(const Fr* points, uint32_t k_i, uint32_t kh, uint32_t kl, Fr* e_hi, Fr* e_lo, const Fr* W, Fr* Wb, Fr* Wc,
                           uint32_t k, uint32_t* dep, uint32_t* host_dep, uint32_t batch, hipStream_t s, uint32_t* wide_bits = nullptr);
enum class LinePart { all, prepare, finish };
void launch_line_restriction(const Fr* W, uint32_t k, const Fr* bc, Fr* scratch, uint32_t* deg_scratch, Fr* bcm, Fr* out, uint32_t* out_len,
                             uint32_t batch, hipStream_t s, LinePart part = LinePart::all);

constexpr uint32_t kWideMinK = 13;
size_t gate_plan_words(uint64_t gates, uint32_t k);
size_t gate_plan_partial_elems(uint64_t gates, uint32_t k);
void launch_gate_plan(GateSpan span, uint32_t k, const uint32_t* offsets, const uint32_t* cursor, const uint32_t* list, uint32_t* plan, hipStream_t s);
struct GateEq {
    const Fr* E;
    const Fr* e_hi;
    const Fr* e_lo_mont;
    uint32_t kl;
};
constexpr uint32_t kGateEqTableMaxKi = 20;
struct GatePlanCounts {
    uint32_t hdr[2][8];
    bool known;
};
size_t gate_plan_arrive_words(uint64_t gates, uint32_t k);
void gate_plan_counts_offsets(uint64_t gates, uint32_t k, size_t* half1_word_offset);
void launch_gate_uv_wide(GateSpan span, uint32_t k_i, uint32_t k, const uint32_t* plan, const GateEq& eq, const Fr* W, Fr* U, Fr* V, LayerBatch lb, Fr* partials,
                         uint32_t* arrive, hipStream_t s, const GateSet* sets = nullptr, const GatePlanCounts* counts = nullptr);
struct WideCFuse {
// ... 112 lines not shown
```

### gkr_amd/csrc/kernels.hip

```cpp
#include <hip/hip_runtime.h>
#include <stdlib.h>

#include <atomic>

#include "kernels.h"
#include "options.h"
#include "dev_util.h"
#include "gate_seg.h"
#include "mfma_fold.h"
#include "mfma_cross.h"
#include "mimc7.h"

namespace gkr {


__device__ __forceinline__ uint64_t mix64(uint64_t z) {
    z = (z ^ (z >> 30)) * 0xBF58476D1CE4E5B9ULL;
    z = (z ^ (z >> 27)) * 0x94D049BB133111EBULL;
    return z ^ (z >> 31);
}

__global__ void k_fill_table(Fr* table, size_t count, uint64_t seed) {
    for (size_t i = blockIdx.x * (size_t)blockDim.x + threadIdx.x; i < count; i += (size_t)gridDim.x * blockDim.x) {
        Fr f;
// ... 210 lines not shown
    }
    __syncthreads();
    if (!s_last) return;
    __threadfence();
    if (threadIdx.x == 0) pub.arrivals[b] = 0u;
    mle_total_and_publish(partials + (size_t)b * nblk, nblk, pub.jout, pub.rec + b, pub.ticket);
}

__global__ void __launch_bounds__(256) k_mle_sub_sums(const Fr* __restrict__ tables, size_t table_stride, uint32_t len,
                                                      MleSubPartial* __restrict__ partials, MlePublish pub) {
    __shared__ Acc<9> smem[4];
    __shared__ uint32_t s_dep;
    const Fr* t = tables + (size_t)blockIdx.y * table_stride;
    const uint32_t chunk = len / gridDim.x;
    const uint32_t begin = blockIdx.x * chunk, end = begin + chunk;
    Acc<9> acc[1] = {acc_zero<9>()};
    uint32_t dep = 0;
    if (threadIdx.x == 0) s_dep = 0;
    __syncthreads();
    for (uint32_t i = begin + threadIdx.x; i < end; i += blockDim.x) {
        const Fr x = load_fr(t + i);
        acc_add_fr(acc[0], x);
        uint32_t d = 0;
#pragma unroll
        for (int k = 0; k < 8; ++k) d |= x.l[k] ^ (uint32_t)__builtin_amdgcn_mov_dpp((int)x.l[k], 0xB1, 0xF, 0xF, true);
        dep |= d;
    }
    if (dep) atomicOr(&s_dep, 1u);
    block_sum<9, 1>(acc, smem);
    if (threadIdx.x == 0) {
        MleSubPartial* p = partials + (size_t)blockIdx.y * gridDim.x + blockIdx.x;
        p->sum = acc[0];
        p->dep = s_dep;
    }
    if (pub.arrivals) mle_publish_from_last_block(partials, pub);
}

__device__ __forceinline__ void half_acc_add(uint32_t (&a)[5], const mf_v4u& x) {
    asm("v_add_co_u32_e32 %0, vcc, %0, %5\n\ts_nop 1\n\t"
        "v_addc_co_u32_e32 %1, vcc, %1, %6, vcc\n\ts_nop 1\n\t"
        "v_addc_co_u32_e32 %2, vcc, %2, %7, vcc\n\ts_nop 1\n\t"
        "v_addc_co_u32_e32 %3, vcc, %3, %8, vcc\n\ts_nop 1\n\t"
        "v_addc_co_u32_e32 %4, vcc, 0, %4, vcc"
        : "+v"(a[0]), "+v"(a[1]), "+v"(a[2]), "+v"(a[3]), "+v"(a[4])
        : "v"(x.x), "v"(x.y), "v"(x.z), "v"(x.w)
        : "vcc");
}

template <int U, int PPW>
__global__ void __launch_bounds__(256) k_mle_sub_sums_stream(const Fr* __restrict__ tables, size_t table_stride, uint32_t chunk, uint32_t nblk,
                                                             MleSubPartial* __restrict__ partials) {
    static_assert(U >= 2 && (U & (U - 1)) == 0, "two sets of U / 2 loads");
    constexpr int H = U / 2;
    const uint32_t lane = threadIdx.x & 63u;
    const uint32_t wave = __builtin_amdgcn_readfirstlane(threadIdx.x >> 6);
    const uint32_t p0 = (blockIdx.x * 4u + wave) * (uint32_t)PPW;
    const uint32_t rpp = chunk / (32u * U);
    const mf_v4u* src = reinterpret_cast<const mf_v4u*>(tables + (size_t)blockIdx.y * table_stride + (size_t)p0 * chunk) + lane;
    MleSubPartial* out = partials + (size_t)blockIdx.y * nblk + p0;

    mf_v4u xa[H], xb[H];
    uint32_t acc[5] = {0u, 0u, 0u, 0u, 0u}, diff = 0u;
    auto load_set = [&](mf_v4u (&x)[H], const mf_v4u* p) {
#pragma unroll
        for (int u = 0; u < H; ++u) x[u] = __builtin_nontemporal_load(p + (size_t)u * 64u);
    };
    auto add_set = [&](const mf_v4u (&x)[H]) {
#pragma unroll
        for (int u = 0; u < H; ++u) {
            half_acc_add(acc, x[u]);
            const mf_v4u v = x[u];
            diff |= (v.x ^ (uint32_t)__builtin_amdgcn_mov_dpp((int)v.x, 0x4E, 0xF, 0xF, true)) |
                    (v.y ^ (uint32_t)__builtin_amdgcn_mov_dpp((int)v.y, 0x4E, 0xF, 0xF, true)) |
                    (v.z ^ (uint32_t)__builtin_amdgcn_mov_dpp((int)v.z, 0x4E, 0xF, 0xF, true)) |
                    (v.w ^ (uint32_t)__builtin_amdgcn_mov_dpp((int)v.w, 0x4E, 0xF, 0xF, true));
        }
    };
    auto finish = [&](MleSubPartial* p) {
        const bool odd = (lane & 1u) != 0u;
        Acc<9> s;
#pragma unroll
        for (int i = 0; i < 4; ++i) {
            s.l[i] = odd ? 0u : acc[i];
            s.l[4 + i] = odd ? acc[i] : (i == 0 ? acc[4] : 0u);
        }
        s.l[8] = odd ? acc[4] : 0u;
        s = wave_sum(s);
        const uint32_t dep = __any(diff != 0u) ? 1u : 0u;
        if (lane == 0) {
            p->sum = s;
            p->dep = dep;
        }
    };

#pragma unroll
    for (int u = 0; u < H; ++u) {
        xa[u] = __builtin_nontemporal_load(src + (size_t)u * 64u);
        __builtin_amdgcn_sched_barrier(0);
    }
#pragma unroll
    for (int u = 0; u < H; ++u) {
        xb[u] = __builtin_nontemporal_load(src + (size_t)(H + u) * 64u);
        __builtin_amdgcn_sched_barrier(0);
    }
    src += (size_t)U * 64u;
    [[maybe_unused]] uint32_t left = rpp;
    for (uint32_t r = (uint32_t)PPW * rpp - 1u; r != 0u; --r) {
        add_set(xa);
        load_set(xa, src);
        __builtin_amdgcn_sched_barrier(0);
        add_set(xb);
        load_set(xb, src + (size_t)H * 64u);
        __builtin_amdgcn_sched_barrier(0);
        src += (size_t)U * 64u;
        if constexpr (PPW > 1) {
            if (--left == 0u) {
                finish(out++);
#pragma unroll
                for (int i = 0; i < 5; ++i) acc[i] = 0u;
                diff = 0u;
                left = rpp;
            }
        }
    }
    add_set(xa);
    add_set(xb);
    finish(out);
}

__device__ __forceinline__ void half_piece_eat(uint32_t (&acc)[5], uint32_t& diff, const mf_v4u& v) {
    half_acc_add(acc, v);
    diff |= (v.x ^ (uint32_t)__builtin_amdgcn_mov_dpp((int)v.x, 0x4E, 0xF, 0xF, true)) |
            (v.y ^ (uint32_t)__builtin_amdgcn_mov_dpp((int)v.y, 0x4E, 0xF, 0xF, true)) |
            (v.z ^ (uint32_t)__builtin_amdgcn_mov_dpp((int)v.z, 0x4E, 0xF, 0xF, true)) |
            (v.w ^ (uint32_t)__builtin_amdgcn_mov_dpp((int)v.w, 0x4E, 0xF, 0xF, true));
}

__device__ __forceinline__ void half_sums_finish(const uint32_t (&acc)[5], uint32_t diff, uint32_t lane, MleSubPartial* p) {
    const bool odd = (lane & 1u) != 0u;
    Acc<9> s;
#pragma unroll
    for (int i = 0; i < 4; ++i) {
        s.l[i] = odd ? 0u : acc[i];
        s.l[4 + i] = odd ? acc[i] : (i == 0 ? acc[4] : 0u);
    }
    s.l[8] = odd ? acc[4] : 0u;
    s = wave_sum(s);
    const uint32_t dep = __any(diff != 0u) ? 1u : 0u;
    if (lane == 0) {
        p->sum = s;
        p->dep = dep;
    }
}

template <int U, int PPW, bool XCD>
__global__ void __launch_bounds__(256) k_mle_sub_sums_roll(const Fr* __restrict__ tables, size_t table_stride, uint32_t chunk, uint32_t nblk,
                                                           MleSubPartial* __restrict__ partials) {
    static_assert(U >= 4 && U % 4 == 0, "the pointer moves once per four pieces");
    const uint32_t lane = threadIdx.x & 63u;
    const uint32_t wave = __builtin_amdgcn_readfirstlane(threadIdx.x >> 6);
    uint32_t bx = blockIdx.x, by = blockIdx.y;
    if constexpr (XCD) {
        const uint32_t nwg = gridDim.x * gridDim.y, L = by * gridDim.x + bx, q = nwg >> 3, r = nwg & 7u, run = L & 7u;
        const uint32_t M = (run < r ? run * (q + 1u) : r * (q + 1u) + (run - r) * q) + (L >> 3);
        by = M / gridDim.x;
        bx = M - by * gridDim.x;
    }
    const uint32_t p0 = (bx * (blockDim.x >> 6) + wave) * (uint32_t)PPW;
    const uint32_t rpp = chunk / (32u * U);
    MleSubPartial* out = partials + (size_t)by * nblk + p0;
    const uint32_t voff = lane * 16u;
    uint64_t next = reinterpret_cast<uint64_t>(tables + (size_t)by * table_stride + (size_t)p0 * chunk);

    mf_v4u x[U];
    uint32_t acc[5] = {0u, 0u, 0u, 0u, 0u}, diff = 0u;
    auto load_step = [&](int u) {
        asm volatile("" : "+s"(next));
        typedef const __attribute__((address_space(1))) mf_v4u* GlobalPiece;
        x[u] = __builtin_nontemporal_load(reinterpret_cast<GlobalPiece>(next + voff) + 64 * (u & 3));
        if ((u & 3) == 3) next += 4096u;
    };
#pragma unroll
    for (int u = 0; u < U; ++u) {
        load_step(u);
        __builtin_amdgcn_sched_barrier(0);
    }
    [[maybe_unused]] uint32_t left = rpp;
    for (uint32_t r = (uint32_t)PPW * rpp - 1u; r != 0u; --r) {
#pragma unroll
        for (int u = 0; u < U; ++u) {
            half_piece_eat(acc, diff, x[u]);
            load_step(u);
            __builtin_amdgcn_sched_barrier(0);
        }
        if constexpr (PPW > 1) {
            if (--left == 0u) {
                half_sums_finish(acc, diff, lane, out++);
#pragma unroll
                for (int i = 0; i < 5; ++i) acc[i] = 0u;
                diff = 0u;
                left = rpp;
            }
        }
    }
#pragma unroll
    for (int u = 0; u < U; ++u) half_piece_eat(acc, diff, x[u]);
    half_sums_finish(acc, diff, lane, out);
}

template <int JIN>
__global__ void __launch_bounds__(256) k_mle_multifold(const Fr* __restrict__ src, size_t src_stride, Fr* __restrict__ dst,
                                                       size_t dst_stride, uint32_t S, const Fr* __restrict__ weights,
                                                       MleSubPartial* __restrict__ partials, MlePublish pub) {
    __shared__ Acc<9> smem[4];
    const Fr* s = src + (size_t)blockIdx.y * src_stride;
    Fr* d = dst + (size_t)blockIdx.y * dst_stride;
    const Fr* w = weights + (size_t)blockIdx.y * kMleMaxSub;
    const uint32_t chunk = S / gridDim.x;
    const uint32_t begin = blockIdx.x * chunk, end = begin + chunk;
    Acc<9> acc[1] = {acc_zero<9>()};
    for (uint32_t i = begin + threadIdx.x; i < end; i += blockDim.x) {
        const Fr y = multifold_entry<JIN>(s, S, i, w);
        store_fr(d + i, y);
        acc_add_fr(acc[0], y);
    }
    block_sum<9, 1>(acc, smem);
    if (threadIdx.x == 0) {
        MleSubPartial* p = partials + (size_t)blockIdx.y * gridDim.x + blockIdx.x;
        p->sum = acc[0];
        p->dep = 0;
    }
    if (pub.arrivals) mle_publish_from_last_block(partials, pub);
}

template <int JIN>
__global__ void __launch_bounds__(1024) k_mle_fold_plan(const Fr* __restrict__ weights, MfmaFoldPlan* __restrict__ plans) {
    __shared__ __attribute__((aligned(16))) unsigned char digits[32 * 32 * (1 << JIN)];
    mfma_plan_block<JIN>(weights + (size_t)blockIdx.x * kMleMaxSub, plans + blockIdx.x, digits);
}

template <int JIN>
__global__ void __launch_bounds__(256) k_mle_multifold_mfma(const Fr* __restrict__ src, size_t src_stride, Fr* __restrict__ dst,
                                                            size_t dst_stride, uint32_t S, const MfmaFoldPlan* __restrict__ plans,
                                                            MleSubPartial* __restrict__ partials, MlePublish pub) {
    __shared__ Acc<9> smem[4];
    __shared__ __attribute__((aligned(16))) unsigned char digits[JIN > 2 ? 32 * 32 * (1 << JIN) : 16];
    const Fr* s = src + (size_t)blockIdx.y * src_stride;
    Fr* d = dst + (size_t)blockIdx.y * dst_stride;
    const uint32_t chunk = S / gridDim.x;
    const uint32_t begin = blockIdx.x * chunk;
    Acc<9> acc[1] = {acc_zero<9>()};
    mfma_multifold_block<JIN>(s, d, S, plans + blockIdx.y, begin, begin + chunk, blockIdx.x * 5u + blockIdx.y * 3u, acc[0], digits);
    block_sum<9, 1>(acc, smem);
    if (threadIdx.x == 0) {
        MleSubPartial* p = partials + (size_t)blockIdx.y * gridDim.x + blockIdx.x;
        p->sum = acc[0];
        p->dep = 0;
    }
    if (pub.arrivals) mle_publish_from_last_block(partials, pub);
}


__global__ void __launch_bounds__(256) k_mle_fine_sums(const MleSubPartial* __restrict__ partials, uint32_t nblk, const Fr* __restrict__ weights,
                                                       MleHostRecSub* __restrict__ host_rec, uint32_t ticket) {
    __shared__ Fr s_w[kMleMaxSub];
    __shared__ Fr s_p[kMleMaxSub][8];
    const uint32_t t = threadIdx.x, q = t >> 5, c = t & 31u, run = nblk >> 10;
    const MleSubPartial* p = partials + (size_t)blockIdx.x * nblk;
    s_w[t >> 3].l[t & 7u] = reinterpret_cast<const uint32_t*>(weights + (size_t)blockIdx.x * kMleMaxSub)[t];
    static_assert(kMleMaxSub * 8 == 256, "one word of the weights per thread");
    __syncthreads();
    Lazy17 dot = lazy_zero();
    for (uint32_t k = 0; k < 4u; ++k) {
        const uint32_t b = q + 8u * k;
        Acc<10> f = acc_zero<10>();
        for (uint32_t i = 0; i < run; ++i) acc_add_acc(f, p[(size_t)(b * 32u + c) * run + i].sum);
        lazy_mac_v(dot, acc_reduce(f), s_w[b]);
    }
    s_p[c][q] = lazy_reduce(dot);
    __syncthreads();
    MleHostRecSub* r = host_rec + blockIdx.x;
    if (t < kMleMaxSub) {
        Acc<9> tot = acc_zero<9>();
        for (uint32_t k = 0; k < 8u; ++k) acc_add_fr(tot, s_p[t][k]);
        r->sums[t] = acc_reduce(tot);
    }
    __syncthreads();
    if (t == 0) __hip_atomic_store(&r->seq, ticket, __ATOMIC_RELEASE, __HIP_MEMORY_SCOPE_SYSTEM);
}

__global__ void __launch_bounds__(256) k_mle_copy_weights(const uint32_t* __restrict__ src, uint32_t* __restrict__ dst) {
    const size_t i = (size_t)blockIdx.x * (8u * kMleMaxSub) + threadIdx.x;
    dst[i] = src[i];
}

__global__ void __launch_bounds__(256, 3) k_mle_multifold2_mfma(const Fr* __restrict__ src, size_t src_stride, Fr* __restrict__ dst, size_t dst_stride,
                                                             uint32_t S, const MfmaFoldPlan* __restrict__ plans, const Fr* __restrict__ w2,
                                                             MleSubPartial* __restrict__ partials, uint32_t T) {
    __shared__ Fr s_prod[2][3][64];
    __shared__ __attribute__((aligned(16))) unsigned char digits[32 * 32 * (1 << kMfmaMaxJ) + 128];
    const Fr* s = src + (size_t)blockIdx.y * src_stride;
    const uint32_t I = S >> kMfmaMaxJ, per = (I >> 6) / T;
    const uint32_t cq = blockIdx.x / per;
    uint32_t it = (blockIdx.x & (per - 1u)) * T;
    const uint32_t lane = threadIdx.x & 63u, wave = (uint32_t)__builtin_amdgcn_readfirstlane((int)(threadIdx.x >> 6));
    const uint32_t begin = 4u * cq * I + 64u * it;
    const Fr wc = load_fr(w2 + (size_t)blockIdx.y * kMleMaxSub + 4u * cq + wave);
    Fr* d = dst + (size_t)blockIdx.y * dst_stride + (size_t)cq * I;
    const uint32_t sub = I >> 5, g = sub < 64u ? sub : 64u;
    MleSubPartial* part = partials + (size_t)blockIdx.y * (8u * (I / g)) + cq;
    mfma_multifold_stream<kMfmaMaxJ, true>(
        s, S, plans + blockIdx.y, begin, begin + 256u * T, 0u, digits,
        [&](uint32_t, uint32_t, uint32_t, const Fr& yw) {
            Lazy17 prod = lazy_zero();
            lazy_mac_s(prod, yw, wc);
            Fr y = lazy_reduce(prod);
            const uint32_t fin = it & 3u, buf = it & 1u;
            if (wave != fin) store_fr(&s_prod[buf][(wave - fin - 1u) & 3u][lane], y);
            __syncthreads();
            if (wave == fin) {
#pragma unroll
                for (int w = 0; w < 3; ++w) y = fr_add(y, load_fr(&s_prod[buf][w][lane]));
                store_fr(d + 64u * it + lane, y);
                Acc<9> acc = acc_zero<9>();
                acc_add_fr(acc, y);
                for (uint32_t off = g >> 1; off >= 1u; off >>= 1) {
                    Acc<9> o;
#pragma unroll
                    for (int l = 0; l < 9; ++l) o.l[l] = __shfl_down(acc.l[l], off, 64);
                    acc_add_acc(acc, o);
                }
                if ((lane & (g - 1u)) == 0u) {
                    MleSubPartial* p = part + (size_t)((64u * it + lane) / g) * 8u;
                    p->sum = acc;
                    p->dep = 0;
                }
            }
            ++it;
            __builtin_amdgcn_sched_barrier(0);
        },
        I, 64u);
}

__global__ void __launch_bounds__(512) k_mle_sub_reduce(const MleSubPartial* __restrict__ partials, uint32_t nblk,
                                                        uint32_t jout, MleHostRecSub* __restrict__ host_rec, uint32_t ticket) {
    mle_total_and_publish(partials + (size_t)blockIdx.x * nblk, nblk, jout, host_rec + blockIdx.x, ticket);
}

__global__ void __launch_bounds__(256) k_mle_sums_small(const Fr* __restrict__ src, size_t src_stride, uint32_t S, uint32_t jout,
                                                        MleHostRecSub* __restrict__ host_rec, uint32_t ticket) {
    const uint32_t b = blockIdx.x;
    const Fr* tbl = src + (size_t)b * src_stride;
    const uint32_t sub = S >> jout, nsub = 1u << jout;
    MleHostRecSub* r = host_rec + b;
    uint32_t dep = 0;
    __shared__ Acc<9> s_part[256];
    const uint32_t tps = 256u >> jout, sb = threadIdx.x / tps, rr = threadIdx.x % tps;
    Acc<9> acc = acc_zero<9>();
    for (uint32_t i = rr; i < sub; i += tps) {
        const Fr x = load_fr(tbl + (size_t)sb * sub + i);
        acc_add_fr(acc, x);
        dep |= fr_eq(x, load_fr(tbl + (((size_t)sb * sub + i) ^ 1u))) ? 0u : 1u;
    }
    s_part[threadIdx.x] = acc;
    __syncthreads();
    for (uint32_t step = tps >> 1; step >= 1u; step >>= 1) {
        if (rr < step) {
            Acc<9> mine = s_part[threadIdx.x];
            acc_add_acc(mine, s_part[threadIdx.x + step]);
            s_part[threadIdx.x] = mine;
        }
        __syncthreads();
    }
    if (threadIdx.x < nsub) r->sums[threadIdx.x] = acc_reduce(s_part[threadIdx.x * tps]);
    dep = __syncthreads_or(dep);
    if (threadIdx.x == 0) {
        r->dep = dep ? 1u : 0u;
        __hip_atomic_store(&r->seq, ticket, __ATOMIC_RELEASE, __HIP_MEMORY_SCOPE_SYSTEM);
    }
}

__global__ void __launch_bounds__(1024) k_mle_multifold_small(const Fr* __restrict__ src, size_t src_stride, Fr* __restrict__ dst,
                                                              size_t dst_stride, uint32_t S, uint32_t jin, uint32_t jout,
                                                              const Fr* __restrict__ weights, MleHostRecSub* __restrict__ host_rec,
                                                              uint32_t ticket, Fr* __restrict__ tail, uint32_t tail_stride, uint32_t planes,
                                                              uint32_t plane_stride) {
    __shared__ Fr s_w[kMleMaxSub];
    extern __shared__ __attribute__((aligned(16))) unsigned char s_y_bytes[];
    Fr* s_y = reinterpret_cast<Fr*>(s_y_bytes);
    __shared__ Acc<9> s_part[kMleMaxSub];
    const uint32_t b = blockIdx.x;
    const Fr* s = src + (size_t)b * src_stride;
    Fr* d = dst + (size_t)b * dst_stride;
    const uint32_t nterm = 1u << jin;
    if (threadIdx.x < nterm * 8u)
        s_w[threadIdx.x >> 3].l[threadIdx.x & 7u] = reinterpret_cast<const uint32_t*>(weights + (size_t)b * kMleMaxSub)[threadIdx.x];
    __syncthreads();
    const uint32_t NT = blockDim.x;
    const uint32_t items = S << jin, per = items > NT ? items / NT : 1u, groups = nterm / per;
    const uint32_t i = threadIdx.x & (S - 1u), q = threadIdx.x / S;
    if (q < groups) {
        Lazy17 acc = lazy_zero();
        for (uint32_t t = 0; t < per; ++t) {
            const uint32_t term = q * per + t;
            Fr x = load_fr(s + (size_t)term * S + i);
            if (planes == kMleFold2Planes) {
                Fr xp[kMleFold2Planes - 1];
#pragma unroll
                for (uint32_t pl = 1; pl < kMleFold2Planes; ++pl) xp[pl - 1] = load_fr(s + (size_t)pl * plane_stride + (size_t)term * S + i);
#pragma unroll
                for (uint32_t pl = 1; pl < kMleFold2Planes; ++pl) x = fr_add(x, xp[pl - 1]);
            }
            lazy_mac_v(acc, x, s_w[term]);
        }
        s_y[q * S + i] = lazy_reduce(acc);
    }
    __syncthreads();
    Fr y;
    if (threadIdx.x < S) {
        Acc<9> tot = acc_zero<9>();
        for (uint32_t g = 0; g < groups; ++g) acc_add_fr(tot, s_y[g * S + threadIdx.x]);
        y = acc_reduce(tot);
        store_fr(d + threadIdx.x, y);
        if (tail) store_fr(tail + (size_t)b * tail_stride + threadIdx.x, y);
    }
    if (tail) __threadfence_system();
    __syncthreads();
    if (threadIdx.x < S) s_y[threadIdx.x] = y;
    __syncthreads();
    const uint32_t nsub = 1u << jout, sub = S >> jout;
    uint32_t tps = NT >> jout;
    if (tps > sub) tps = sub;
    const uint32_t sb = threadIdx.x / tps, rr = threadIdx.x % tps;
    MleHostRecSub* r = host_rec + b;
    const bool mine = sb < nsub;
    Acc<9> acc = acc_zero<9>();
    if (mine)
        for (uint32_t k = rr; k < sub; k += tps) acc_add_fr(acc, s_y[sb * sub + k]);
    const uint32_t within = tps < 64u ? tps : 64u;
    for (uint32_t off = within >> 1; off >= 1u; off >>= 1) {
        Acc<9> o;
#pragma unroll
        for (int l = 0; l < 9; ++l) o.l[l] = __shfl_down(acc.l[l], off, 64);
        acc_add_acc(acc, o);
    }
    if (tps > 64u) {
        __shared__ Acc<9> s_wave[16];
        if (mine && (threadIdx.x & 63u) == 0) s_wave[threadIdx.x >> 6] = acc;
        __syncthreads();
        if (threadIdx.x < nsub) {
            Acc<9> tot = acc_zero<9>();
            for (uint32_t w = 0; w < (tps >> 6); ++w) acc_add_acc(tot, s_wave[threadIdx.x * (tps >> 6) + w]);
            s_part[threadIdx.x] = tot;
        }
    } else if (mine && rr == 0) {
        s_part[sb] = acc;
    }
    __syncthreads();
    if (threadIdx.x < nsub) r->sums[threadIdx.x] = acc_reduce(s_part[threadIdx.x]);
    __syncthreads();
    if (threadIdx.x == 0) {
        r->dep = 0u;
        __hip_atomic_store(&r->seq, ticket, __ATOMIC_RELEASE, __HIP_MEMORY_SCOPE_SYSTEM);
    }
}

__global__ void __launch_bounds__(256) k_mle_fold_sum_small(const Fr* __restrict__ src, size_t src_stride,
                                                            Fr* __restrict__ dst, size_t dst_stride, uint32_t q,
                                                            const FixedMul* __restrict__ rtab,
                                                            MleHostRec* __restrict__ host_rec, uint32_t ticket) {
    __shared__ Acc<9> smem[4 * 2];
    const uint32_t b = blockIdx.x;
    const Fr* s = src + (size_t)b * src_stride;
    Fr* d = dst + (size_t)b * dst_stride;
    const FixedMul T = rtab[b];
    Acc<9> acc[2] = {acc_zero<9>(), acc_zero<9>()};
    for (uint32_t i = threadIdx.x; i < q; i += blockDim.x) {
        Fr x0 = load_fr(s + i), x1 = load_fr(s + i + 2 * (size_t)q);
        Fr x2 = load_fr(s + i + q), x3 = load_fr(s + i + 3 * (size_t)q);
        Fr y0 = fr_fold_fixed(x0, x1, T);
        Fr y1 = fr_fold_fixed(x2, x3, T);
        store_fr(d + i, y0);
        store_fr(d + i + q, y1);
        acc_add_fr(acc[0], y0);
        acc_add_fr(acc[1], y1);
    }
    block_sum<9, 2>(acc, smem);
    if (threadIdx.x == 0) {
// ... 1588 lines not shown
            const uint32_t ablocks = (uint32_t)((a + kScanPerBlock - 1) / kScanPerBlock), bblocks = (uint32_t)((b + kScanPerBlock - 1) / kScanPerBlock);
            uint32_t *cnt = seg_scratch, *off = cnt + a, *asums = off + a, *lh = asums + ablocks + 1, *ls = lh + b, *bsums = ls + b,
                     *csums = bsums + bblocks + 1;
            segs->shift = p.shift;
            segs->runs = p.runs;
            segs->run_base = p.run_base;
            segs->bound = p.bound;
            segs->half_bound = p.half_bound;
            segs->groups = p.groups;
            segs->nb = 1u << k;
            segs->packed_half = p.packed_half;
            const dim3 sg((unsigned)((a + 255) / 256));
            hipLaunchKernelGGL(k_seg_count, sg, dim3(256), 0, s, starts, hist, lblocks, p.m, p.runs, p.nseg, cnt);
            hipLaunchKernelGGL(k_scan_blocks, dim3(ablocks), dim3(256), 0, s, cnt, off, asums, a);
            hipLaunchKernelGGL(k_scan_sums, dim3(1), dim3(1024), 0, s, asums, ablocks);
            hipLaunchKernelGGL(k_scan_add, dim3(ablocks), dim3(256), 0, s, off, (uint32_t*)nullptr, asums, a);
            hipLaunchKernelGGL(k_seg_fill, sg, dim3(256), 0, s, starts, hist, lblocks, p.m, p.runs, p.nseg, off, segs->items(), segs->bucket_begin());
            const uint32_t per = (p.bound + p.len_blocks - 1) / p.len_blocks;
            hipLaunchKernelGGL(k_seg_len_hist, dim3(p.len_blocks), dim3(256), 0, s, segs->items(), segs->bucket_begin(), 1u << k, per, lh);
            hipLaunchKernelGGL(k_scan_blocks, dim3(bblocks), dim3(256), 0, s, lh, ls, bsums, b);
            hipLaunchKernelGGL(k_scan_sums, dim3(1), dim3(1024), 0, s, bsums, bblocks);
            hipLaunchKernelGGL(k_scan_add, dim3(bblocks), dim3(256), 0, s, ls, (uint32_t*)nullptr, bsums, b);
            hipLaunchKernelGGL(k_seg_len_fill, dim3(p.len_blocks), dim3(256), 0, s, segs->items(), segs->bucket_begin(), 1u << k, per, ls, segs->order());
            const size_t c = 2 * (size_t)p.groups + 1;
            const uint32_t cblocks = (uint32_t)((c + kScanPerBlock - 1) / kScanPerBlock);
            hipLaunchKernelGGL(k_seg_group_len, dim3((unsigned)((c + 255) / 256)), dim3(256), 0, s, segs->items(), segs->order(), segs->bucket_begin(),
                               1u << k, p.groups, segs->group_len());
            hipLaunchKernelGGL(k_scan_blocks, dim3(cblocks), dim3(256), 0, s, segs->group_len(), segs->group_off(), csums, c);
            hipLaunchKernelGGL(k_scan_sums, dim3(1), dim3(1024), 0, s, csums, cblocks);
            hipLaunchKernelGGL(k_scan_add, dim3(cblocks), dim3(256), 0, s, segs->group_off(), (uint32_t*)nullptr, csums, c);
            hipLaunchKernelGGL(k_seg_pack, dim3((2 * p.groups + 3) / 4), dim3(256), 0, s, segs->items(), segs->order(), segs->bucket_begin(), 1u << k, p.groups,
                               segs->group_len(), segs->group_off(), list, list + gate_list_words(gates), (uint32_t)span.base, p.shift,
                               segs->packed());
        }
        return;
    }
    const uint32_t gblocks = blocks_for(gates, 4096);
    const uint32_t sblocks = (uint32_t)((n + kScanPerBlock - 1) / kScanPerBlock);
    hipLaunchKernelGGL(k_gate_count, dim3(gblocks), dim3(256), 0, s, gates, k, gate_type, left, right, counts, bad);
    hipLaunchKernelGGL(k_scan_blocks, dim3(sblocks), dim3(256), 0, s, counts, offsets, block_sums, n);
    hipLaunchKernelGGL(k_scan_sums, dim3(1), dim3(1024), 0, s, block_sums, sblocks);
    hipLaunchKernelGGL(k_scan_add, dim3(sblocks), dim3(256), 0, s, offsets, cursor, block_sums, n);
    hipLaunchKernelGGL(k_gate_fill, dim3(gblocks), dim3(256), 0, s, gates, k, gate_type, left, right, cursor, list, list + gate_list_words(gates));
}

static uint32_t device_cus() {
    static std::atomic<uint32_t> cus[64];
    int dev = 0;
    if (hipGetDevice(&dev) != hipSuccess) return 256u;
    std::atomic<uint32_t>& slot = cus[dev & 63];
    uint32_t n = slot.load(std::memory_order_relaxed);
    if (!n) {
        hipDeviceProp_t prop;
        n = (hipGetDeviceProperties(&prop, dev) == hipSuccess && prop.multiProcessorCount >= 1) ? (uint32_t)prop.multiProcessorCount : 256u;
        slot.store(n, std::memory_order_relaxed);
    }
    return n;
}
template <bool ROWS, bool LDS_T>
static void launch_seg_pass_t(const GateSegs& g, uint32_t k, const Fr* e_lo_mont, const Fr* T, Fr* X, Fr* Y, LayerBatch lb, hipStream_t s) {
    const uint32_t tlen = 1u << k;
    const size_t lds = LDS_T ? (size_t)tlen * sizeof(Fr) : 0;
    static std::atomic<uint64_t> attr_set{0};
    int dev = 0;
    (void)hipGetDevice(&dev);
    if (LDS_T && !((attr_set.load(std::memory_order_relaxed) >> (dev & 63)) & 1u)) {
        if (hipFuncSetAttribute(reinterpret_cast<const void*>(&k_seg_pass<ROWS, LDS_T>), hipFuncAttributeMaxDynamicSharedMemorySize, 160 * 1024) != hipSuccess) {
            (void)hipGetLastError();
            launch_seg_pass_t<ROWS, false>(g, k, e_lo_mont, T, X, Y, lb, s);
            return;
        }
        attr_set.fetch_or((uint64_t)1 << (dev & 63), std::memory_order_relaxed);
    }
    const uint32_t blocks = LDS_T ? device_cus() : 4 * device_cus();
    hipLaunchKernelGGL((k_seg_pass<ROWS, LDS_T>), dim3(blocks, lb.batch), dim3(LDS_T ? 1024 : 256), lds, s, g.items(), g.order(), g.bucket_begin(),
                       g.nb, g.groups, g.group_len(), g.group_off(), g.packed(), e_lo_mont, g.shift, T, tlen,
                       (uint32_t)lb.wstride, X, Y, g.half_bound);
}
static void launch_seg_pass(bool rows, const GateSegs& g, uint32_t k, const Fr* e_lo_mont, const Fr* T, Fr* X, Fr* Y, LayerBatch lb, hipStream_t s) {
    const bool no_lds = opt(OPT_gate_segments_no_lds) != 0;
    const bool lds_t = !no_lds && ((size_t)sizeof(Fr) << k) <= 128 * 1024;
    if (rows)
        lds_t ? launch_seg_pass_t<true, true>(g, k, e_lo_mont, T, X, Y, lb, s) : launch_seg_pass_t<true, false>(g, k, e_lo_mont, T, X, Y, lb, s);
    else
        lds_t ? launch_seg_pass_t<false, true>(g, k, e_lo_mont, T, X, Y, lb, s) : launch_seg_pass_t<false, false>(g, k, e_lo_mont, T, X, Y, lb, s);
}

void launch_exclusive_scan(const uint32_t* in, uint32_t* out, uint32_t* block_sums, size_t n, hipStream_t s) {
    const uint32_t sblocks = (uint32_t)((n + kScanPerBlock - 1) / kScanPerBlock);
    hipLaunchKernelGGL(k_scan_blocks, dim3(sblocks), dim3(256), 0, s, in, out, block_sums, n);
    hipLaunchKernelGGL(k_scan_sums, dim3(1), dim3(1024), 0, s, block_sums, sblocks);
    hipLaunchKernelGGL(k_scan_add, dim3(sblocks), dim3(256), 0, s, out, (uint32_t*)nullptr, block_sums, n);
}

static uint32_t bucket_threads(uint64_t gates, uint32_t k) { return (gates >> k) > 64u ? 256u : 64u; }

void launch_gate_uv(GateSpan span, uint32_t k_i, uint32_t k, const uint32_t* offsets, const uint32_t* cursor, const uint32_t* list,
                    const Fr* e_hi, const Fr* e_lo_mont, uint32_t kl, const Fr* W, Fr* U, Fr* V, LayerBatch lb, const GateSegs* segs,
                    Fr* partials, hipStream_t s, const GateSet* sets) {
    if (segs && segs->shift && partials && !sets) {
        Fr *X = partials, *Y = partials + (size_t)segs->half_bound * lb.batch;
        launch_seg_pass(false, *segs, k, e_lo_mont, W, X, Y, lb, s);
        hipLaunchKernelGGL(k_seg_combine, dim3(((1u << k) + 1u) / 2u, lb.batch), dim3(64), 0, s, segs->items(), segs->bucket_begin(), 0u, 1u << k, X, Y,
                           segs->half_bound, e_hi, k_i - segs->shift, segs->run_base, U, V, (uint32_t)lb.wstride, CPhaseFuse{});
        return;
    }
    hipLaunchKernelGGL(k_gate_uv, dim3(1u << k, lb.batch), dim3(bucket_threads(span.count, k)), 0, s, offsets, cursor, list,
                       list + gate_list_words(span.count), e_hi, e_lo_mont, kl, k_i - kl, W, U, V, (uint32_t)lb.wstride, (uint32_t)span.base, sets);
}

bool launch_gate_rows(GateSpan span, uint32_t k_i, uint32_t k, const uint32_t* offsets, const uint32_t* cursor, const uint32_t* list,
                      const Fr* e_hi, const Fr* e_lo_mont, uint32_t kl, const Fr* eq_mont, Fr* A_row, Fr* M_row, LayerBatch lb,
                      const GateSegs* segs, Fr* partials, hipStream_t s, const CPhaseFuse* fuse, const GateSet* sets) {
    if (segs && segs->shift && partials && !sets) {
        Fr *X = partials, *Y = partials + (size_t)segs->half_bound * lb.batch;
        launch_seg_pass(true, *segs, k, e_lo_mont, eq_mont, X, Y, lb, s);
        hipLaunchKernelGGL(k_seg_combine, dim3(((1u << k) + 1u) / 2u, lb.batch), dim3(64), 0, s, segs->items(), segs->bucket_begin(), 1u << k, 1u << k, X, Y,
                           segs->half_bound, e_hi, k_i - segs->shift, segs->run_base, A_row, M_row, (uint32_t)lb.wstride, fuse ? *fuse : CPhaseFuse{});
        return fuse != nullptr;
    }
    hipLaunchKernelGGL(k_gate_rows, dim3(1u << k, lb.batch), dim3(bucket_threads(span.count, k)), 0, s, offsets, cursor, list,
                       list + gate_list_words(span.count), e_hi, e_lo_mont, kl, k_i - kl, eq_mont, A_row, M_row, k, (uint32_t)lb.wstride,
                       (uint32_t)span.base, sets);
    return false;
}

void launch_predicate_normalise(const unsigned long long* wide, Fr* out, size_t cells, hipStream_t s) {
    hipLaunchKernelGGL(k_predicate_normalise, dim3(blocks_for(cells, 4096)), dim3(256), 0, s, wide, out, cells);
}

void launch_mle_fold_sum_small(const Fr* src, size_t src_stride, Fr* dst, size_t dst_stride, uint32_t q, uint32_t batch,
                               const FixedMul* rtab, MleHostRec* host_rec, uint32_t ticket, hipStream_t s) {
    hipLaunchKernelGGL(k_mle_fold_sum_small, dim3(batch), dim3(256), 0, s, src, src_stride, dst, dst_stride, q, rtab,
                       host_rec, ticket);
}

uint32_t mle_pass_blocks(uint32_t items, uint32_t jout, uint32_t batch) {
    uint32_t want = mle_blocks_per_table(items, batch);
    uint32_t b = 1u << jout;
    while (b < want && b * 2 <= items && b * 2 <= kMaxBlocksPerTable) b <<= 1;
    if (b > items) b = items;
    return b;
}

static int mle_sub_sums_stream_form(uint32_t len, uint32_t batch, uint32_t nblk, bool publishes) {
    const long long o = opt(OPT_pass0_stream);
    const long long want = o >= 1 && o <= 3 ? o : kMlePass0Stream;
    if (want < 2 || publishes || nblk == 0 || len % nblk != 0) return 0;
    const uint32_t chunk = len / nblk;
    if (chunk % 512u == 0 && nblk % 8u == 0 && (uint64_t)batch * nblk >= kMlePass0DeepMinPartials) return want == 3 ? 3 : 2;
    return chunk % 256u == 0 && nblk % 4u == 0 ? 1 : 0;
}

void launch_mle_sub_sums(const Fr* tables, size_t stride, uint32_t len, uint32_t batch, uint32_t nblk, MleSubPartial* partials,
                         hipStream_t s, const MlePublish* publish) {
    const int form = mle_sub_sums_stream_form(len, batch, nblk, publish != nullptr);
    if (form == 3)
        hipLaunchKernelGGL((k_mle_sub_sums_roll<16, 1, true>), dim3(nblk / 4u, batch), dim3(256), 0, s, tables, stride, len / nblk, nblk, partials);
    else if (form == 2)
        hipLaunchKernelGGL((k_mle_sub_sums_stream<16, 2>), dim3(nblk / 8u, batch), dim3(256), 0, s, tables, stride, len / nblk, nblk, partials);
    else if (form == 1)
        hipLaunchKernelGGL((k_mle_sub_sums_stream<8, 1>), dim3(nblk / 4u, batch), dim3(256), 0, s, tables, stride, len / nblk, nblk, partials);
    else
        hipLaunchKernelGGL(k_mle_sub_sums, dim3(nblk, batch), dim3(256), 0, s, tables, stride, len, partials, publish ? *publish : MlePublish{});
}

void launch_mle_sub_reduce(const MleSubPartial* partials, uint32_t nblk, uint32_t jout, uint32_t batch, MleHostRecSub* host_rec,
                           uint32_t ticket, hipStream_t s) {
    hipLaunchKernelGGL(k_mle_sub_reduce, dim3(batch), dim3(512), 0, s, partials, nblk, jout, host_rec, ticket);
}

bool mle_multifold_uses_mfma(uint32_t S, uint32_t nblk) {
    const bool off = opt(OPT_no_mfma_fold) != 0;
    return !off && nblk > 0 && S % nblk == 0 && (S / nblk) % 64u == 0;
}

size_t mle_fold_plan_bytes() { return sizeof(MfmaFoldPlan); }

void launch_mle_fold_plan(int jin, const Fr* weights, void* plans, uint32_t batch, hipStream_t s, uint32_t threads) {
    MfmaFoldPlan* pl = static_cast<MfmaFoldPlan*>(plans);
    if (jin == 1)
        hipLaunchKernelGGL(k_mle_fold_plan<1>, dim3(batch), dim3(64), 0, s, weights, pl);
    else if (jin == 2)
        hipLaunchKernelGGL(k_mle_fold_plan<2>, dim3(batch), dim3(128), 0, s, weights, pl);
    else if (jin == 3)
        hipLaunchKernelGGL(k_mle_fold_plan<3>, dim3(batch), dim3(256), 0, s, weights, pl);
    else if (jin == 4)
        hipLaunchKernelGGL(k_mle_fold_plan<4>, dim3(batch), dim3(512), 0, s, weights, pl);
    else
        hipLaunchKernelGGL(k_mle_fold_plan<5>, dim3(batch), dim3(threads ? threads : 1024u), 0, s, weights, pl);
}

void launch_mle_multifold(int jin, const Fr* src, size_t src_stride, Fr* dst, size_t dst_stride, uint32_t S, uint32_t batch,
                          uint32_t nblk, const Fr* weights, const void* plans, MleSubPartial* partials, hipStream_t s,
                          const MlePublish* publish) {
    dim3 grid(nblk, batch);
    const MlePublish pub = publish ? *publish : MlePublish{};
    if (mle_multifold_uses_mfma(S, nblk)) {
        const MfmaFoldPlan* pl = static_cast<const MfmaFoldPlan*>(plans);
        if (jin == 1)
            hipLaunchKernelGGL(k_mle_multifold_mfma<1>, grid, dim3(256), 0, s, src, src_stride, dst, dst_stride, S, pl, partials, pub);
        else if (jin == 2)
            hipLaunchKernelGGL(k_mle_multifold_mfma<2>, grid, dim3(256), 0, s, src, src_stride, dst, dst_stride, S, pl, partials, pub);
        else if (jin == 3)
            hipLaunchKernelGGL(k_mle_multifold_mfma<3>, grid, dim3(256), 0, s, src, src_stride, dst, dst_stride, S, pl, partials, pub);
        else if (jin == 4)
            hipLaunchKernelGGL(k_mle_multifold_mfma<4>, grid, dim3(256), 0, s, src, src_stride, dst, dst_stride, S, pl, partials, pub);
        else
            hipLaunchKernelGGL(k_mle_multifold_mfma<5>, grid, dim3(256), 0, s, src, src_stride, dst, dst_stride, S, pl, partials, pub);
        return;
    }
    if (jin == 1)
        hipLaunchKernelGGL(k_mle_multifold<1>, grid, dim3(256), 0, s, src, src_stride, dst, dst_stride, S, weights, partials, pub);
    else if (jin == 2)
        hipLaunchKernelGGL(k_mle_multifold<2>, grid, dim3(256), 0, s, src, src_stride, dst, dst_stride, S, weights, partials, pub);
    else
        hipLaunchKernelGGL(k_mle_multifold<3>, grid, dim3(256), 0, s, src, src_stride, dst, dst_stride, S, weights, partials, pub);
}

uint32_t mle_multifold_blocks(uint32_t S, uint32_t jout, uint32_t batch) {
    const bool off = opt(OPT_no_mfma_fold) != 0;
    if (off) return mle_pass_blocks(S, jout, batch);
    const uint32_t target = opt(OPT_fold_blocks) > 0 ? (uint32_t)opt(OPT_fold_blocks) : 65536u;
    const uint32_t mc = (uint32_t)opt(OPT_fold_min_chunk);
    const uint32_t min_chunk = mc >= 64u && (mc & (mc - 1u)) == 0 ? mc : 256u;
    uint32_t b = 1u << jout;
    while ((uint64_t)b * batch < target && S / (2u * b) >= min_chunk && 2u * b <= kMaxBlocksPerTable) b <<= 1;
    if (b > S) b = S;
    return b;
}

void launch_mle_multifold_small(int jin, const Fr* src, size_t src_stride, Fr* dst, size_t dst_stride, uint32_t S, uint32_t jout,
                                uint32_t batch, const Fr* weights, MleHostRecSub* host_rec, uint32_t ticket, hipStream_t s, Fr* tail, uint32_t tail_stride,
                                uint32_t planes, uint32_t plane_stride) {
    dim3 grid(batch);
    const uint32_t threads = planes > 1 && S <= 256u ? 256u : 1024u;
    if (jin == 0)
        hipLaunchKernelGGL(k_mle_sums_small, grid, dim3(256), 0, s, src, src_stride, S, jout, host_rec, ticket);
    else
        hipLaunchKernelGGL(k_mle_multifold_small, grid, dim3(threads), threads * sizeof(Fr), s, src, src_stride, dst, dst_stride, S, (uint32_t)jin, jout, weights,
                           host_rec, ticket, tail, tail_stride, planes, plane_stride);
}

uint32_t mle_multifold2_partials(uint32_t S) {
    const uint32_t I = S >> kMfmaMaxJ, sub = I >> 5;
    return 8u * (I / (sub < 64u ? sub : 64u));
}

void launch_mle_fine_sums(const MleSubPartial* partials, uint32_t nblk, const Fr* weights, uint32_t batch, MleHostRecSub* host_rec, uint32_t ticket,
                          hipStream_t s) {
    hipLaunchKernelGGL(k_mle_fine_sums, dim3(batch), dim3(256), 0, s, partials, nblk, weights, host_rec, ticket);
}

void launch_mle_copy_weights(const Fr* src, Fr* dst, uint32_t batch, hipStream_t s) {
    hipLaunchKernelGGL(k_mle_copy_weights, dim3(batch), dim3(8 * kMleMaxSub), 0, s, reinterpret_cast<const uint32_t*>(src),
                       reinterpret_cast<uint32_t*>(dst));
}

uint32_t mle_multifold2_tiles(uint32_t S) {
    const uint32_t tiles = S >> 11;
    const long long want = opt(OPT_fold2_tiles);
    uint32_t T = 1;
    while (2u * T <= tiles && 2ll * T <= want) T <<= 1;
    return T;
}

void launch_mle_multifold2(const Fr* src, size_t src_stride, Fr* dst, size_t dst_stride, uint32_t S, uint32_t batch, const void* plans, const Fr* w2,
                           MleSubPartial* partials, hipStream_t s) {
    const uint32_t T = mle_multifold2_tiles(S);
    hipLaunchKernelGGL(k_mle_multifold2_mfma, dim3((S >> 8) / T, batch), dim3(256), 0, s, src, src_stride, dst, dst_stride, S,
                       static_cast<const MfmaFoldPlan*>(plans), w2, partials, T);
}

void launch_mle_round_reduce(const MlePartial* partials, uint32_t nblk, uint32_t batch, MleHostRec* host_rec,
                             uint32_t ticket, hipStream_t s) {
    hipLaunchKernelGGL(k_mle_round_reduce, dim3(batch), dim3(64), 0, s, partials, nblk, host_rec, ticket);
}


}
```

### gkr_amd/csrc/options.h

```cpp
#pragma once
#include <stdlib.h>
#include <string.h>

namespace gkr {

#define GKR_CONTEXT_OPTIONS(X)                                                                                                       \
                                                                  \
    X(rounds_per_pass, "rounds_per_pass", "GKR_ROUNDS_PER_PASS", 0, "rounds a pass of the plain sumcheck covers (0: 5; 3 without the MFMA fold)") \
    X(no_mfma_fold, "no_mfma_fold", "GKR_NO_MFMA_FOLD", 0, "fold passes on v_mad_u64_u32 instead of int8 MFMA")                      \
    X(first_fold_levels, "first_fold_levels", "GKR_FIRST_FOLD_LEVELS", 0, "variables the first fold of a host-hashed 2^18 .. 2^24-point sumcheck binds: 1 five, 2 ten in the one read (0: the default, capi_internal.h kMleFirstFoldLevels)") \
    X(pass0_stream, "pass0_stream", "GKR_PASS0_STREAM", 0, "pass 0 of a streaming launch of the plain sumcheck: 1 k_mle_sub_sums (a block per partial), 2 its pipelined form (a wave per one or two partials, 16-byte loads kept in flight in two sets) where it applies, 3 as 2 with the rolling form (a wave per partial, ONE buffer of sixteen loads, every XCD on a contiguous eighth of the launch) in place of the form of two partials per wave (0: the default, kernels.h kMlePass0Stream)") \
    X(fold2_tiles, "fold2_tiles", "GKR_FOLD2_TILES", 0, "64-entry tiles a block of the two-level first fold takes: k forces min(k, 2^(n-16)), a power of two (0: one, which is fastest where measured)") \
    X(no_fused_reduce, "no_fused_reduce", "GKR_NO_FUSED_REDUCE", 0, "latency-bound passes publish through k_mle_sub_reduce instead of from their last block") \
    X(hash_chunk, "hash_chunk", "GKR_HASH_CHUNK", 0, "8 or 16: sumchecks per host hash call (0: 16 when host threads are scarce)")    \
    X(device_hash_percent, "device_hash_percent", "GKR_DEVICE_HASH_PERCENT", 0, "share of a batch of >= 64 plain sumchecks hashed on the device (0..90)") \
    X(group_size, "group_size", "GKR_GROUP_SIZE", 0, "sumchecks per scheduling group of a batch (0: groups of ~4 GiB of tables)")     \
    X(pass_queue_depth, "pass_queue_depth", "GKR_PASS_QUEUE_DEPTH", 0, "groups whose pass 0 is queued up front (0: two)")           \
    X(no_late_stream, "no_late_stream", "GKR_NO_LATE_STREAM", 0, "a group's small late passes stay on the main stream")              \
    X(plan_main, "plan_main", "GKR_PLAN_MAIN", 0, "the fold plan (digit matrix) on the main stream instead of the side stream")       \
    X(mle_per_round, "mle_per_round", "GKR_MLE_PER_ROUND", 0, "one variable per pass (the first schedule; what the device transcript uses)") \
    X(fold_blocks, "fold_blocks", "GKR_FOLD_BLOCKS", 0, "target block count of a fold pass (0: 65536)")                              \
    X(fold_min_chunk, "fold_min_chunk", "GKR_FOLD_MIN_CHUNK", 0, "smallest chunk of entries per fold block (0: 256)")                \
    X(items_per_block, "items_per_block", "GKR_ITEMS_PER_BLOCK", 0, "entries per block of the first pass (0: 1024)")                 \
                                                                \
    X(predicate_atomics, "predicate_atomics", "GKR_PREDICATE_ATOMICS", 0, "dense predicate tables by widened-atomic scatter instead of the counting sort") \
    X(gate_groups_min_k, "gate_groups_min_k", "GKR_GATE_GROUPS_MIN_K", -1, "smallest k_next whose layers take the wide layers' item passes (-1: 13)") \
    X(no_fused_publish, "no_fused_publish", "GKR_NO_FUSED_PUBLISH", 0, "product passes publish through a second launch instead of from their last block") \
    X(gate_sort_global, "gate_sort_global", "GKR_GATE_SORT_GLOBAL", 0, "the gate lists' counting sort with global atomics where the LDS sort applies") \
    X(gate_segments_off, "gate_segments_off", "GKR_GATE_SEGMENTS_OFF", 0, "bucket kernels instead of the segment passes on large layers") \
    X(gate_segments_min_log2, "gate_segments_min_log2", "GKR_GATE_SEGMENTS_MIN_LOG2", 22, "smallest layer (log2 gates) that takes the segment passes") \
    X(gate_segment_log2, "gate_segment_log2", "GKR_GATE_SEGMENT_LOG2", 0, "log2 of the segments' mean length (0: 4)")              \
    X(gate_segments_no_lds, "gate_segments_no_lds", "GKR_GATE_SEGMENTS_NO_LDS", 0, "the segment pass gathers its table from L2 instead of LDS") \
    X(no_mfma_cross, "no_mfma_cross", "GKR_NO_MFMA_CROSS", 0, "wide layers' product passes over tables of 2^15 entries and more on v_mad_u64_u32 instead of int8 MFMA") \
    X(prod_cross_min_log2, "prod_cross_min_log2", "GKR_PROD_CROSS_MIN_LOG2", 0, "smallest tables (log2 entries, at least 13) whose cross sums of a product pass run on the matrix cores (0: 15)") \
    X(prod_fold_min_log2, "prod_fold_min_log2", "GKR_PROD_FOLD_MIN_LOG2", 0, "smallest tables (log2 entries) whose pending fold of a product pass runs on the matrix cores (0: 17)") \
    X(host_tail_log2, "host_tail_log2", "GKR_HOST_TAIL_LOG2", 0, "a phase's product passes over tables of 2^this entries and fewer run on the host (0: 6; -1: none; at most 12)") \
    X(host_tail_max_batch, "host_tail_max_batch", "GKR_HOST_TAIL_MAX_BATCH", 0, "largest batch (proofs advancing together) whose small product passes run on the host (0: 8)") \
    X(line_stepwise, "line_stepwise", "GKR_LINE_STEPWISE", 0, "q_i in its wide-layer form (one launch per variable) at every width")  \
    X(layer_no_fused, "layer_no_fused", "GKR_LAYER_NO_FUSED", 0, "device transcript: separate fold and sum kernels in the b-phase")   \
                                  \
    X(no_circuit_cache, "no_circuit_cache", "GKR_NO_CIRCUIT_CACHE", 0, "do not keep proven circuits' gate arrays and lists on the device between calls") \
    X(prove_many_pieces, "prove_many_pieces", "GKR_PROVE_MANY_PIECES", 0, "gkr_prove_many: cut the costliest items in two until there are this many")      \
    X(prove_many_lockstep, "prove_many_lockstep", "GKR_PROVE_MANY_LOCKSTEP", 1, "gkr_prove_many: items whose circuits share a k list advance in lockstep, one launch per pass for the group (0: one chain per item)") \
    X(lockstep_max_proofs, "lockstep_max_proofs", "GKR_LOCKSTEP_MAX_PROOFS", 0, "most proofs one lockstep group may hold (0: 32 -- beyond that independent chains overlap better)") \
                                                                \
    X(verify_workspace_mb, "verify_workspace_mb", "GKR_VERIFY_WORKSPACE_MB", 0, "gkr_verify_prepared / gkr_sumcheck_mle_verify*: MiB of device workspace a chunk of proofs may take (0: 2048; a chunk is never less than one proof)") \
    X(verify_device_hash_min, "verify_device_hash_min", "GKR_VERIFY_DEVICE_HASH_MIN", 0, "gkr_verify_prepared / gkr_sumcheck_mle_verify*: smallest number of round vectors in a chunk whose challenge hashes run on the device (0: the measured default, capi_verify.hip kVerifyDeviceHashMinRows; -1: never, the host threads hash; 1: always)") \
                         \
    X(mle_eval_mfma_min_n, "mle_eval_mfma_min_n", "GKR_MLE_EVAL_MFMA_MIN_N", 0, "gkr_mle_eval_batch_device / gkr_sumcheck_mle_verify*: smallest n whose tables are evaluated by the streaming matrix-core kernel (0: the default, kernels.h kMleEvalMfmaMinN; never below 11, where the kernel starts to apply; above 24: the one-block kernel up to n = 24, its largest)")

enum OptionId : int {
#define GKR_OPT_ENUM(id, name, env, def, doc) OPT_##id,
    GKR_CONTEXT_OPTIONS(GKR_OPT_ENUM)
#undef GKR_OPT_ENUM
        OPT_COUNT
};

struct OptionInfo {
    const char* name;
    const char* env;
    long long def;
    const char* doc;
};

inline const OptionInfo* option_table() {
    static const OptionInfo table[OPT_COUNT] = {
#define GKR_OPT_ROW(id, name, env, def, doc) {name, env, def, doc},
        GKR_CONTEXT_OPTIONS(GKR_OPT_ROW)
#undef GKR_OPT_ROW
    };
    return table;
}

struct Options {
    long long v[OPT_COUNT];
    static Options from_environment() {
        Options o;
        const OptionInfo* t = option_table();
        for (int i = 0; i < OPT_COUNT; ++i) {
            o.v[i] = t[i].def;
            if (const char* e = getenv(t[i].env)) {
                char* end = nullptr;
                const long long val = strtoll(e, &end, 0);
                o.v[i] = end != e ? val : 1;
            }
        }
        return o;
    }
};

inline int option_index(const char* name) {
    if (!name) return -1;
    const OptionInfo* t = option_table();
    for (int i = 0; i < OPT_COUNT; ++i)
        if (!strcmp(t[i].name, name) || !strcmp(t[i].env, name)) return i;
    return -1;
}

inline const Options*& current_options() {
    static thread_local const Options* cur = nullptr;
    return cur;
}
inline const Options& default_options() {
    static const Options d = Options::from_environment();
    return d;
}
inline long long opt(OptionId id) {
    const Options* o = current_options();
    return (o ? o : &default_options())->v[id];
}
struct OptionScope {
    const Options* prev;
    explicit OptionScope(const Options* o) : prev(current_options()) { current_options() = o; }
    ~OptionScope() { current_options() = prev; }
    OptionScope(const OptionScope&) = delete;
    OptionScope& operator=(const OptionScope&) = delete;
};

inline bool process_switch(const char* env) { return getenv(env) != nullptr; }
inline int process_int(const char* env, int def) {
    const char* e = getenv(env);
    return e ? atoi(e) : def;
}
inline bool debug_timing() {
    static const bool on = process_switch("GKR_DEBUG_TIMING");
    return on;
}

}
```

Baseline: 501.8 billion.

## Publish streaming-pass partials as flagged records to pinned memory, totalled on host

The rolling pass 0 and the two-level first fold now write per-block partial sums straight to pinned host memory as flag-in-word records tagged with a ticket. Idle hashing threads scan and total these records, which removes the k_mle_sub_reduce launch between consecutive streaming launches. Later passes on other streams are ordered behind the publishing pass with events recorded on demand. In exchange the kernels do extra PCIe stores, the host spends time polling, and the cross-stream ordering logic becomes considerably more complex.

```diff
diff --git a/gkr_amd/csrc/capi_internal.h b/gkr_amd/csrc/capi_internal.h
--- a/gkr_amd/csrc/capi_internal.h
+++ b/gkr_amd/csrc/capi_internal.h
@@ -239,6 +239,7 @@
     hipStream_t late = nullptr;
     hipStream_t chain = nullptr;
     std::vector<hipEvent_t> aux_events;
+    std::vector<hipEvent_t> ended_events;
     Fr* d_cts = nullptr;
     int transcript = GKR_TRANSCRIPT_HOST;
     std::string err;
@@ -338,6 +339,16 @@
         return hipSuccess;
     }
 
+    hipError_t stream_end_events(int events) {
+        while ((int)ended_events.size() < events) {
+            hipEvent_t e;
+            hipError_t rc = hipEventCreateWithFlags(&e, hipEventDisableTiming | hipEventDisableSystemFence);
+            if (rc != hipSuccess) return rc;
+            ended_events.push_back(e);
+        }
+        return hipSuccess;
+    }
+
     int fail(int status, const std::string& what) {
         err = what;
         return status;
diff --git a/gkr_amd/csrc/capi_mle_passes.hip b/gkr_amd/csrc/capi_mle_passes.hip
--- a/gkr_amd/csrc/capi_mle_passes.hip
+++ b/gkr_amd/csrc/capi_mle_passes.hip
@@ -59,6 +59,8 @@
     gkr::MleHostRecSub* rec = nullptr;
     uint32_t* arrivals = nullptr;
     Fr* h_tail = nullptr;
+    uint64_t* h_flag = nullptr;
+    uint64_t* flag_rec(int b) const { return h_flag + (size_t)b * gkr::kFlagRecsPerTable * gkr::kFlagRecWords; }
 };
 static int mle_pass_tables(gkr_ctx* ctx, const std::string& prefix, const Fr* input, size_t len, size_t work_len, int batch, MlePassTables& T) {
     T.input = input;
@@ -102,6 +104,7 @@
     Fr* export_tail = nullptr;
     int blocks_jout = 0;
     uint32_t src_planes = 1;
+    bool flagged = false;
 };
 static uint32_t pass0_blocks(size_t len, int jout, int nb, const MlePassPolicy& P) {
     uint32_t nblk = gkr::mle_pass_blocks((uint32_t)len, (uint32_t)(P.blocks_jout > 0 ? P.blocks_jout : jout), nb);
@@ -112,23 +115,26 @@
     Timed t(ctx, "mle_sub_reduce", 0.0, st, true);
     gkr::launch_mle_sub_reduce(T.partials + (size_t)b0 * gkr::kMaxBlocksPerTable, nblk, (uint32_t)jout, nb, T.rec + b0, ticket, st);
 }
-static void queue_pass0(gkr_ctx* ctx, const MlePassTables& T, int b0, int nb, int jout, uint32_t ticket, hipStream_t st, const MlePassPolicy& P) {
+static bool queue_pass0(gkr_ctx* ctx, const MlePassTables& T, int b0, int nb, int jout, uint32_t ticket, hipStream_t st, const MlePassPolicy& P) {
     const size_t len = T.in_stride;
     const Fr* src = T.input + (size_t)b0 * len;
     const double bytes = (double)nb * len * 32.0;
     if (len <= gkr::kSmallPassEntries) {
         Timed t(ctx, "mle_pass_small", bytes, st, true);
         gkr::launch_mle_multifold_small(0, src, len, nullptr, 0, (uint32_t)len, (uint32_t)jout, nb, T.h_w + (size_t)b0 * gkr::kMleMaxSub, T.rec + b0, ticket, st);
-        return;
+        return false;
     }
     const uint32_t nblk = pass0_blocks(len, jout, nb, P);
     gkr::MlePublish pub;
     const bool fused = fused_publish(T, b0, nb, nblk, bytes, ticket, jout, pub);
+    bool flagged;
     {
         Timed t(ctx, P.row, bytes, st, fused);
-        gkr::launch_mle_sub_sums(src, len, (uint32_t)len, nb, nblk, T.partials + (size_t)b0 * gkr::kMaxBlocksPerTable, st, fused ? &pub : nullptr);
-    }
-    if (!fused) queue_sub_reduce(ctx, T, b0, nb, nblk, jout, ticket, st);
+        flagged = gkr::launch_mle_sub_sums(src, len, (uint32_t)len, nb, nblk, T.partials + (size_t)b0 * gkr::kMaxBlocksPerTable, st, fused ? &pub : nullptr,
+                                           P.flagged && !fused ? T.flag_rec(b0) : nullptr, ticket);
+    }
+    if (!fused && !flagged) queue_sub_reduce(ctx, T, b0, nb, nblk, jout, ticket, st);
+    return flagged;
 }
 static void queue_fold(gkr_ctx* ctx, const MlePassTables& T, int b0, int nb, bool from_input, int m_src, int jin, int jout, uint32_t ticket,
                        hipStream_t st, const MlePassPolicy& P) {
@@ -224,6 +230,15 @@
     hipStream_t chain = nullptr;
     bool on_host = false;
     bool mid = false, planes = false;
+    std::atomic<uint32_t> flag_ticket{0};
+    std::atomic<int> flag_left{0};
+    int pub_index = -1;
+    bool end_bound = false;
+};
+struct FlagScan {
+    std::atomic<uint32_t> busy{0};
+    std::atomic<uint32_t> done{0};
+    std::atomic<uint32_t> cursor{0}, cursor_ticket{0};
 };
 struct MlePassClock {
     const bool on = gkr::debug_timing();
@@ -253,6 +268,15 @@
     std::vector<PassGroup> grp;
     std::vector<uint32_t> dep_last;
     int next_first = 0;
+    int folds_queued = 0;
+    struct PubLaunch {
+        int b0;
+        uint32_t ticket;
+    };
+    std::vector<PubLaunch> pubs;
+    int pubs_started = -1;
+    hipError_t order_err = hipSuccess;
+    std::unique_ptr<FlagScan[]> scan;
     gkr_fr *stage_c = nullptr, *stage_r = nullptr;
     uint32_t* stage_len = nullptr;
     MlePassClock clock;
@@ -262,14 +286,40 @@
         G.m -= jin;
         G.round0 += jin;
         G.j = rounds_for(G.m);
-        G.ticket = ++ctx->ticket;
+        G.ticket = gkr::next_ticket(ctx->ticket);
+    }
+    void arm_totals(PassGroup& G, bool end_bound) {
+        G.pub_index = (int)pubs.size();
+        G.end_bound = end_bound;
+        pubs.push_back({G.b0, G.ticket});
+        G.flag_left.store(G.nb, std::memory_order_relaxed);
+        G.flag_ticket.store(G.ticket, std::memory_order_release);
+    }
+    hipEvent_t ended_event(const PassGroup& G) const { return ctx->ended_events[G.index]; }
+    bool later_launch_started(int index) {
+        for (int q = (int)pubs.size() - 1; q > index && q > pubs_started; --q)
+            if ((uint32_t)(__atomic_load_n(T.flag_rec(pubs[q].b0), __ATOMIC_RELAXED) >> 32) == pubs[q].ticket) pubs_started = q;
+        return pubs_started > index;
+    }
+    void after_stream_pass(PassGroup& G, hipStream_t st) {
+        const int index = G.pub_index;
+        G.pub_index = -1;
+        if (index < 0 || st == s) return;
+        hipError_t e = hipSuccess;
+        if (!G.end_bound) {
+            if (later_launch_started(index) || hipStreamQuery(s) == hipSuccess) return;
+            e = hipEventRecord(ended_event(G), s);
+        }
+        if (e == hipSuccess) e = hipStreamWaitEvent(st, ended_event(G), 0);
+        if (e != hipSuccess && order_err == hipSuccess) order_err = e;
     }
     void launch_first(PassGroup& G) {
-        G.ticket = ++ctx->ticket;
+        G.ticket = gkr::next_ticket(ctx->ticket);
         MlePassPolicy P;
         P.row = G.chain ? "mle_sub_sums_dev" : "mle_sub_sums";
         if (two_level(G)) P.blocks_jout = kMleTwoLevelRounds;
-        queue_pass0(ctx, T, G.b0, G.nb, G.j, G.ticket, G.chain ? G.chain : s, P);
+        P.flagged = scan && two_level(G) && G.j == gkr::kMlePassMaxRounds;
+        if (queue_pass0(ctx, T, G.b0, G.nb, G.j, G.ticket, G.chain ? G.chain : s, P)) arm_totals(G, false);
     }
     void launch_next_first() {
         if (next_first < sc.groups) launch_first(grp[next_first++]);
@@ -278,6 +328,7 @@
         const int m_src = G.m;
         const bool from_input = m_src == n;
         hipStream_t st = G.chain ? G.chain : ((!from_input && m_src <= 16) ? late : s);
+        after_stream_pass(G, st);
         advance(G, jin);
         MlePassPolicy P;
         P.row = G.chain ? "mle_multifold_dev" : (st == s ? "mle_multifold" : "mle_multifold_late");
@@ -294,12 +345,13 @@
         const int J = G.j;
         G.mid = true;
         G.round0 += J;
-        G.ticket = ++ctx->ticket;
+        G.ticket = gkr::next_ticket(ctx->ticket);
         hipStream_t side = side_launches() ? ctx->aux : s;
         MlePassPolicy P0;
         P0.blocks_jout = kMleTwoLevelRounds;
         const uint32_t nblk0 = pass0_blocks(T.in_stride, J, G.nb, P0);
         const Fr* w = T.h_w + (size_t)G.b0 * gkr::kMleMaxSub;
+        after_stream_pass(G, side);
         Timed t(ctx, "mle_fold_plan", 0.0, side, true);
         gkr::launch_mle_fine_sums(T.partials + (size_t)G.b0 * gkr::kMaxBlocksPerTable, nblk0, w, G.nb, T.rec + G.b0, G.ticket, side);
         gkr::launch_mle_fold_plan(J, w, T.plans + (size_t)G.b0 * gkr::mle_fold_plan_bytes(), G.nb, side, side == s ? 0u : 256u);
@@ -321,14 +373,63 @@
         G.m = n - kMleTwoLevelRounds;
         G.round0 += G.j;
         G.j = gkr::kMlePassMaxRounds;
-        G.ticket = ++ctx->ticket;
+        G.ticket = gkr::next_ticket(ctx->ticket);
+        ++folds_queued;
+        const bool last_streaming = next_first == sc.groups && folds_queued == sc.groups;
+        const bool before_last = scan && folds_queued == sc.groups - 1;
+        bool flagged;
         {
             Timed t(ctx, "mle_multifold", (double)G.nb * ((double)T.in_stride + (double)(gkr::kMleFold2Planes * (S >> gkr::kMlePassMaxRounds))) * 32.0, s);
-            gkr::launch_mle_multifold2(T.input + (size_t)G.b0 * T.in_stride, T.in_stride, T.work + (size_t)G.b0 * T.work_len, T.work_len, S, G.nb,
-                                       T.plans + (size_t)G.b0 * gkr::mle_fold_plan_bytes(), T.d_w2 + (size_t)G.b0 * gkr::kMleMaxSub,
-                                       T.partials + (size_t)G.b0 * gkr::kMaxBlocksPerTable, s);
-        }
-        queue_sub_reduce(ctx, T, G.b0, G.nb, npart, G.j, G.ticket, s);
+            flagged = gkr::launch_mle_multifold2(T.input + (size_t)G.b0 * T.in_stride, T.in_stride, T.work + (size_t)G.b0 * T.work_len, T.work_len, S, G.nb,
+                                                 T.plans + (size_t)G.b0 * gkr::mle_fold_plan_bytes(), T.d_w2 + (size_t)G.b0 * gkr::kMleMaxSub,
+                                                 T.partials + (size_t)G.b0 * gkr::kMaxBlocksPerTable, s, scan && !last_streaming ? T.flag_rec(G.b0) : nullptr,
+                                                 G.ticket, before_last ? ended_event(G) : nullptr);
+        }
+        if (flagged)
+            arm_totals(G, before_last);
+        else
+            queue_sub_reduce(ctx, T, G.b0, G.nb, npart, G.j, G.ticket, s);
+    }
+    bool try_total() {
+        if (!scan) return false;
+        constexpr uint32_t kWords = gkr::kFlagRecsPerTable * gkr::kFlagRecWords;
+        for (int g = 0; g < sc.groups; ++g) {
+            PassGroup& G = grp[g];
+            const uint32_t t = G.flag_ticket.load(std::memory_order_acquire);
+            if (!t) continue;
+            for (int b = G.b0; b < G.b0 + G.nb; ++b) {
+                FlagScan& F = scan[b];
+                if (F.done.load(std::memory_order_relaxed) == t || F.busy.load(std::memory_order_relaxed)) continue;
+                const uint32_t at = F.cursor_ticket.load(std::memory_order_relaxed) == t ? F.cursor.load(std::memory_order_relaxed) : 0u;
+                if (at < kWords && (uint32_t)(__atomic_load_n(T.flag_rec(b) + at, __ATOMIC_RELAXED) >> 32) != t) continue;
+                if (F.busy.exchange(1u, std::memory_order_acquire)) continue;
+                bool totalled = false;
+                if (F.done.load(std::memory_order_relaxed) != t) {
+                    uint32_t cursor = F.cursor_ticket.load(std::memory_order_relaxed) == t ? F.cursor.load(std::memory_order_relaxed) : 0u;
+                    gkr::MleHostRecSub& R = T.h_rec[b];
+                    uint32_t dep = 0;
+                    static_assert(sizeof(R.sums) == gkr::kMleMaxSub * 32, "a sum is four 64-bit words");
+                    const bool landed = gkr::flagged_scan(T.flag_rec(b), kWords, t, &cursor);
+                    F.cursor.store(cursor, std::memory_order_relaxed);
+                    F.cursor_ticket.store(t, std::memory_order_relaxed);
+                    if (landed &&
+                        gkr::flagged_total(T.flag_rec(b), gkr::kFlagRecsPerTable, gkr::kMleMaxSub, t, reinterpret_cast<uint64_t*>(R.sums), &dep)) {
+                        R.dep = dep;
+                        __atomic_store_n(&R.seq, t, __ATOMIC_RELEASE);
+                        F.done.store(t, std::memory_order_relaxed);
+                        totalled = true;
+                    }
+                }
+                F.busy.store(0u, std::memory_order_release);
+                if (!totalled) continue;
+                if (G.flag_left.fetch_sub(1, std::memory_order_acq_rel) == 1) {
+                    uint32_t expect = t;
+                    G.flag_ticket.compare_exchange_strong(expect, 0u, std::memory_order_acq_rel);
+                }
+                return true;
+            }
+        }
+        return false;
     }
     void host_fold(PassGroup& G, int jin) {
         using gkr::h64::F;
@@ -376,7 +477,7 @@
             uint32_t best_gen = 0;
             for (int g = 0; g < sc.groups; ++g)
                 if (const uint32_t gen = grp[g].open_generation(); gen && (best < 0 || gen < best_gen)) best = g, best_gen = gen;
-            if (best < 0) return false;
+            if (best < 0) return try_total();
             PassGroup& G = grp[best];
             uint32_t first, take;
             if (!G.try_claim(sc.chunk[best], &first, &take)) continue;
@@ -448,7 +549,9 @@
         while (active > 0 && rc == GKR_OK) {
             bool progress = false;
             for (int g = 0; g < next_first; ++g) progress |= step(grp[g], active);
-            if (progress)
+            if (order_err != hipSuccess)
+                rc = ctx->hip_fail(order_err, "ordering a launch behind a publishing pass");
+            else if (progress)
                 rc = watch.progressed();
             else if (!try_work())
                 rc = watch.idled();
@@ -472,7 +575,12 @@
         HIP_TRY(ctx, ctx->pinned_host("mlep.w2", sizeof(Fr) * gkr::kMleMaxSub * batch, reinterpret_cast<void**>(&R.T.h_w2)));
         WS(ctx, "mlep.d_w2", Fr, (size_t)batch * gkr::kMleMaxSub, R.T.d_w2);
     }
+    if (gkr::opt(gkr::OPT_stream_publish) != 1 && sc.two_level && sc.groups > 1) {
+        HIP_TRY(ctx, ctx->pinned_host("mlep.flag", sizeof(uint64_t) * gkr::kFlagRecWords * gkr::kFlagRecsPerTable * batch, reinterpret_cast<void**>(&R.T.h_flag)));
+        R.scan.reset(new FlagScan[batch]);
+    }
     HIP_TRY(ctx, ctx->aux_stream(sc.groups));
+    if (R.scan) HIP_TRY(ctx, ctx->stream_end_events(sc.groups));
     if (sc.tail_on) HIP_TRY(ctx, ctx->pinned_host("mlep.tail", sizeof(Fr) * ((size_t)batch << kMleTailLog2), reinterpret_cast<void**>(&R.T.h_tail)));
     if (!gkr::opt(gkr::OPT_no_late_stream) && sc.groups > 1) HIP_TRY(ctx, ctx->late_stream(&R.late));
     R.dep_last = std::vector<uint32_t>(batch, 0);
@@ -581,7 +689,7 @@
         run_pieces(pool, &work_fn, batch > 16);
     }
     void pass(bool pass0, bool from_input, int m_src, int jin, int J, int round0) {
-        const uint32_t ticket = ++ctx->ticket;
+        const uint32_t ticket = gkr::next_ticket(ctx->ticket);
         if (!rc) {
             MlePassPolicy P;
             P.row = pass0 ? "mle_sub_sums" : "mle_multifold";
@@ -655,7 +763,7 @@
     if (folded) {
         MlePassPolicy P;
         P.row = "mle_multifold";
-        queue_fold(ctx, T, 0, batch, round0 == jin, m + jin, jin, 1, ++ctx->ticket, s, P);
+        queue_fold(ctx, T, 0, batch, round0 == jin, m + jin, jin, 1, gkr::next_ticket(ctx->ticket), s, P);
         if (hipError_t le = hipGetLastError(); le != hipSuccess) R.rc = ctx->hip_fail(le, "launch of the last rank-local fold");
     }
     R.gather_tail(folded ? T.work : T.input, folded ? T.work_len : len, m, lp, shard, d_tail);
diff --git a/gkr_amd/csrc/flagged_rec.h b/gkr_amd/csrc/flagged_rec.h
--- /dev/null
+++ b/gkr_amd/csrc/flagged_rec.h
@@ -0,0 +1,63 @@
+#pragma once
+#include <stdint.h>
+
+#include "fr64.h"
+
+namespace gkr {
+
+constexpr uint32_t kFlagRecWords = 10;
+constexpr uint32_t kFlagRecsPerTable = 256;
+
+inline uint64_t flag_word(uint32_t data, uint32_t ticket) { return ((uint64_t)ticket << 32) | data; }
+
+inline uint32_t next_ticket(uint32_t& counter) {
+    if (++counter == 0u) ++counter;
+    return counter;
+}
+
+inline bool flagged_scan(const uint64_t* words, uint32_t nwords, uint32_t ticket, uint32_t* cursor) {
+    uint32_t c = *cursor;
+    while (c < nwords && (uint32_t)(__atomic_load_n(words + c, __ATOMIC_RELAXED) >> 32) == ticket) ++c;
+    *cursor = c;
+    return c == nwords;
+}
+
+inline h64::F flagged_reduce(h64::F lo, uint64_t hi) {
+    while (h64::geq_mod(lo)) h64::sub_mod(lo);
+    return h64::add(lo, h64::to_mont(h64::F{{hi, 0, 0, 0}}));
+}
+
+inline bool flagged_total(const uint64_t* words, uint32_t nrec, uint32_t nsub, uint32_t ticket, uint64_t* sums, uint32_t* dep) {
+    const uint32_t per = nrec / nsub;
+    uint32_t d = 0;
+    for (uint32_t s = 0; s < nsub; ++s) {
+        uint64_t limb[kFlagRecWords - 1] = {0, 0, 0, 0, 0, 0, 0, 0, 0};
+        for (uint32_t k = 0; k < per; ++k) {
+            const uint64_t* rec = words + (size_t)(s * per + k) * kFlagRecWords;
+            for (uint32_t l = 0; l < kFlagRecWords; ++l) {
+                const uint64_t w = __atomic_load_n(rec + l, __ATOMIC_RELAXED);
+                if ((uint32_t)(w >> 32) != ticket) return false;
+                if (l + 1 < kFlagRecWords)
+                    limb[l] += (uint32_t)w;
+                else
+                    d |= (uint32_t)w;
+            }
+        }
+        uint32_t v[kFlagRecWords];
+        uint64_t carry = 0;
+        for (uint32_t l = 0; l + 1 < kFlagRecWords; ++l) {
+            const uint64_t t = limb[l] + carry;
+            v[l] = (uint32_t)t;
+            carry = t >> 32;
+        }
+        v[kFlagRecWords - 1] = (uint32_t)carry;
+        h64::F lo;
+        for (int i = 0; i < 4; ++i) lo.l[i] = (uint64_t)v[2 * i] | ((uint64_t)v[2 * i + 1] << 32);
+        const h64::F r = flagged_reduce(lo, (uint64_t)v[8] | ((uint64_t)v[9] << 32));
+        for (int i = 0; i < 4; ++i) sums[4 * s + i] = r.l[i];
+    }
+    *dep = d ? 1u : 0u;
+    return true;
+}
+
+}
diff --git a/gkr_amd/csrc/gkr_capi.hip b/gkr_amd/csrc/gkr_capi.hip
--- a/gkr_amd/csrc/gkr_capi.hip
+++ b/gkr_amd/csrc/gkr_capi.hip
@@ -84,6 +84,7 @@
     ctx->release_buffers();
     if (ctx->d_cts) (void)hipFree(ctx->d_cts);
     for (hipEvent_t e : ctx->aux_events) (void)hipEventDestroy(e);
+    for (hipEvent_t e : ctx->ended_events) (void)hipEventDestroy(e);
     if (ctx->aux) (void)hipStreamDestroy(ctx->aux);
     if (ctx->late) (void)hipStreamDestroy(ctx->late);
     if (ctx->chain) (void)hipStreamDestroy(ctx->chain);
diff --git a/gkr_amd/csrc/kernels.h b/gkr_amd/csrc/kernels.h
--- a/gkr_amd/csrc/kernels.h
+++ b/gkr_amd/csrc/kernels.h
@@ -1,8 +1,10 @@
 #pragma once
+#include <hip/hip_ext.h>
 #include <hip/hip_runtime.h>
 #include <stddef.h>
 #include <stdint.h>
 
+#include "flagged_rec.h"
 #include "fr32.h"
 
 namespace gkr {
@@ -94,8 +96,8 @@
 bool mle_multifold_uses_mfma(uint32_t S, uint32_t nblk);
 constexpr int kMlePass0Stream = 3;
 constexpr uint64_t kMlePass0DeepMinPartials = 2u * 12u * 256u * 4u;
-void launch_mle_sub_sums(const Fr* tables, size_t stride, uint32_t len, uint32_t batch, uint32_t nblk, MleSubPartial* partials,
-                         hipStream_t s, const MlePublish* publish = nullptr);
+bool launch_mle_sub_sums(const Fr* tables, size_t stride, uint32_t len, uint32_t batch, uint32_t nblk, MleSubPartial* partials,
+                         hipStream_t s, const MlePublish* publish = nullptr, uint64_t* flagged = nullptr, uint32_t flag_ticket = 0);
 void launch_mle_sub_reduce(const MleSubPartial* partials, uint32_t nblk, uint32_t jout, uint32_t batch, MleHostRecSub* host_rec,
                            uint32_t ticket, hipStream_t s);
 size_t mle_fold_plan_bytes();
@@ -115,8 +117,8 @@
 void launch_mle_fine_sums(const MleSubPartial* partials, uint32_t nblk, const Fr* weights, uint32_t batch, MleHostRecSub* host_rec, uint32_t ticket,
                           hipStream_t s);
 void launch_mle_copy_weights(const Fr* src, Fr* dst, uint32_t batch, hipStream_t s);
-void launch_mle_multifold2(const Fr* src, size_t src_stride, Fr* dst, size_t dst_stride, uint32_t S, uint32_t batch, const void* plans, const Fr* w2,
-                           MleSubPartial* partials, hipStream_t s);
+bool launch_mle_multifold2(const Fr* src, size_t src_stride, Fr* dst, size_t dst_stride, uint32_t S, uint32_t batch, const void* plans, const Fr* w2,
+                           MleSubPartial* partials, hipStream_t s, uint64_t* flagged = nullptr, uint32_t flag_ticket = 0, hipEvent_t ended = nullptr);
 void launch_layer_round_reduce(const LayerPartial* partials, uint32_t nblk, LayerHostRec* host_rec, uint32_t ticket,
                                LayerBatch lb, hipStream_t s);
 void launch_fold_small(Fr* W, uint32_t hw, const FixedMul* rtab, LayerBatch lb, hipStream_t s);
diff --git a/gkr_amd/csrc/kernels.hip b/gkr_amd/csrc/kernels.hip
--- a/gkr_amd/csrc/kernels.hip
+++ b/gkr_amd/csrc/kernels.hip
@@ -386,6 +386,21 @@
         p->dep = dep;
     }
 }
+__device__ __forceinline__ void half_sums_total(const uint32_t (&acc)[5], uint32_t diff, uint32_t lane, Acc<9>& s, uint32_t& dep) {
+    const bool odd = (lane & 1u) != 0u;
+#pragma unroll
+    for (int i = 0; i < 4; ++i) {
+        s.l[i] = odd ? 0u : acc[i];
+        s.l[4 + i] = odd ? acc[i] : (i == 0 ? acc[4] : 0u);
+    }
+    s.l[8] = odd ? acc[4] : 0u;
+    s = wave_sum(s);
+    dep = __any(diff != 0u) ? 1u : 0u;
+}
+
+__device__ __forceinline__ void mle_flag_store(uint64_t* p, uint32_t data, uint32_t ticket) {
+    __hip_atomic_store(p, ((uint64_t)ticket << 32) | data, __ATOMIC_RELAXED, __HIP_MEMORY_SCOPE_SYSTEM);
+}
 
 template <int U, int PPW, bool XCD>
 __global__ void __launch_bounds__(256) k_mle_sub_sums_roll(const Fr* __restrict__ tables, size_t table_stride, uint32_t chunk, uint32_t nblk,
@@ -440,6 +455,77 @@
 #pragma unroll
     for (int u = 0; u < U; ++u) half_piece_eat(acc, diff, x[u]);
     half_sums_finish(acc, diff, lane, out);
+}
+
+template <int U, bool XCD>
+__global__ void __launch_bounds__(256) k_mle_sub_sums_roll_pub(const Fr* __restrict__ tables, size_t table_stride, uint32_t chunk, uint32_t nblk,
+                                                               MleSubPartial* __restrict__ partials, uint64_t* __restrict__ flagged, uint32_t ticket) {
+    static_assert(U >= 4 && U % 4 == 0, "the pointer moves once per four pieces");
+    __shared__ uint32_t s_pub[4][kFlagRecWords];
+    const uint32_t lane = threadIdx.x & 63u;
+    const uint32_t wave = __builtin_amdgcn_readfirstlane(threadIdx.x >> 6);
+    uint32_t bx = blockIdx.x, by = blockIdx.y;
+    if constexpr (XCD) {
+        const uint32_t nwg = gridDim.x * gridDim.y, L = by * gridDim.x + bx, q = nwg >> 3, r = nwg & 7u, run = L & 7u;
+        const uint32_t M = (run < r ? run * (q + 1u) : r * (q + 1u) + (run - r) * q) + (L >> 3);
+        by = M / gridDim.x;
+        bx = M - by * gridDim.x;
+    }
+    const uint32_t p0 = bx * 4u + wave;
+    const uint32_t rpp = chunk / (32u * U);
+    MleSubPartial* out = partials + (size_t)by * nblk + p0;
+    const uint32_t voff = lane * 16u;
+    uint64_t next = reinterpret_cast<uint64_t>(tables + (size_t)by * table_stride + (size_t)p0 * chunk);
+
+    mf_v4u x[U];
+    uint32_t acc[5] = {0u, 0u, 0u, 0u, 0u}, diff = 0u;
+    auto load_step = [&](int u) {
+        asm volatile("" : "+s"(next));
+        typedef const __attribute__((address_space(1))) mf_v4u* GlobalPiece;
+        x[u] = __builtin_nontemporal_load(reinterpret_cast<GlobalPiece>(next + voff) + 64 * (u & 3));
+        if ((u & 3) == 3) next += 4096u;
+    };
+#pragma unroll
+    for (int u = 0; u < U; ++u) {
+        load_step(u);
+        __builtin_amdgcn_sched_barrier(0);
+    }
+    for (uint32_t r = rpp - 1u; r != 0u; --r) {
+#pragma unroll
+        for (int u = 0; u < U; ++u) {
+            half_piece_eat(acc, diff, x[u]);
+            load_step(u);
+            __builtin_amdgcn_sched_barrier(0);
+        }
+    }
+#pragma unroll
+    for (int u = 0; u < U; ++u) half_piece_eat(acc, diff, x[u]);
+    Acc<9> s;
+    uint32_t dep;
+    half_sums_total(acc, diff, lane, s, dep);
+    if (lane == 0) {
+        out->sum = s;
+        out->dep = dep;
+#pragma unroll
+        for (int l = 0; l < 9; ++l) s_pub[wave][l] = s.l[l];
+        s_pub[wave][9] = dep;
+    }
+    __syncthreads();
+    if (wave == 0 && lane < kFlagRecWords) {
+        Acc<9> tot = acc_zero<9>();
+        uint32_t d = 0;
+        for (uint32_t w = 0; w < 4u; ++w) {
+            Acc<9> o;
+#pragma unroll
+            for (int l = 0; l < 9; ++l) o.l[l] = s_pub[w][l];
+            acc_add_acc(tot, o);
+            d |= s_pub[w][9];
+        }
+        uint32_t word = d;
+#pragma unroll
+        for (int l = 0; l < 9; ++l) word = lane == (uint32_t)l ? tot.l[l] : word;
+        mle_flag_store(flagged + ((size_t)by * (nblk / 4u) + bx) * kFlagRecWords + lane, word, ticket);
+    }
 }
 
 template <int JIN>
@@ -528,9 +614,11 @@
     dst[i] = src[i];
 }
 
+template <bool PUB>
 __global__ void __launch_bounds__(256, 3) k_mle_multifold2_mfma(const Fr* __restrict__ src, size_t src_stride, Fr* __restrict__ dst, size_t dst_stride,
                                                              uint32_t S, const MfmaFoldPlan* __restrict__ plans, const Fr* __restrict__ w2,
-                                                             MleSubPartial* __restrict__ partials, uint32_t T) {
+                                                             MleSubPartial* __restrict__ partials, uint32_t T, uint64_t* __restrict__ flagged,
+                                                             uint32_t ticket) {
     __shared__ Fr s_prod[2][3][64];
     __shared__ __attribute__((aligned(16))) unsigned char digits[32 * 32 * (1 << kMfmaMaxJ) + 128];
     const Fr* s = src + (size_t)blockIdx.y * src_stride;
@@ -568,6 +656,17 @@
                     MleSubPartial* p = part + (size_t)((64u * it + lane) / g) * 8u;
                     p->sum = acc;
                     p->dep = 0;
+                }
+                if constexpr (PUB) {
+                    const uint32_t from = lane & ~(g - 1u), wl = lane & (g - 1u);
+                    uint32_t word = 0u;
+#pragma unroll
+                    for (int l = 0; l < 9; ++l) {
+                        const uint32_t v = __shfl(acc.l[l], from, 64);
+                        word = wl == (uint32_t)l ? v : word;
+                    }
+                    if (wl < kFlagRecWords)
+                        mle_flag_store(flagged + ((size_t)blockIdx.y * kFlagRecsPerTable + ((64u * it + from) / g) * 8u + cq) * kFlagRecWords + wl, word, ticket);
                 }
             }
             ++it;
@@ -2462,9 +2561,14 @@
     return chunk % 256u == 0 && nblk % 4u == 0 ? 1 : 0;
 }
 
-void launch_mle_sub_sums(const Fr* tables, size_t stride, uint32_t len, uint32_t batch, uint32_t nblk, MleSubPartial* partials,
-                         hipStream_t s, const MlePublish* publish) {
+bool launch_mle_sub_sums(const Fr* tables, size_t stride, uint32_t len, uint32_t batch, uint32_t nblk, MleSubPartial* partials,
+                         hipStream_t s, const MlePublish* publish, uint64_t* flagged, uint32_t flag_ticket) {
     const int form = mle_sub_sums_stream_form(len, batch, nblk, publish != nullptr);
+    if (form == 3 && flagged && nblk == 4u * kFlagRecsPerTable) {
+        hipLaunchKernelGGL((k_mle_sub_sums_roll_pub<16, true>), dim3(nblk / 4u, batch), dim3(256), 0, s, tables, stride, len / nblk, nblk, partials, flagged,
+                           flag_ticket);
+        return true;
+    }
     if (form == 3)
         hipLaunchKernelGGL((k_mle_sub_sums_roll<16, 1, true>), dim3(nblk / 4u, batch), dim3(256), 0, s, tables, stride, len / nblk, nblk, partials);
     else if (form == 2)
@@ -2473,6 +2577,7 @@
         hipLaunchKernelGGL((k_mle_sub_sums_stream<8, 1>), dim3(nblk / 4u, batch), dim3(256), 0, s, tables, stride, len / nblk, nblk, partials);
     else
         hipLaunchKernelGGL(k_mle_sub_sums, dim3(nblk, batch), dim3(256), 0, s, tables, stride, len, partials, publish ? *publish : MlePublish{});
+    return false;
 }
 
 void launch_mle_sub_reduce(const MleSubPartial* partials, uint32_t nblk, uint32_t jout, uint32_t batch, MleHostRecSub* host_rec,
@@ -2575,11 +2680,18 @@
     return T;
 }
 
-void launch_mle_multifold2(const Fr* src, size_t src_stride, Fr* dst, size_t dst_stride, uint32_t S, uint32_t batch, const void* plans, const Fr* w2,
-                           MleSubPartial* partials, hipStream_t s) {
+bool launch_mle_multifold2(const Fr* src, size_t src_stride, Fr* dst, size_t dst_stride, uint32_t S, uint32_t batch, const void* plans, const Fr* w2,
+                           MleSubPartial* partials, hipStream_t s, uint64_t* flagged, uint32_t flag_ticket, hipEvent_t ended) {
     const uint32_t T = mle_multifold2_tiles(S);
-    hipLaunchKernelGGL(k_mle_multifold2_mfma, dim3((S >> 8) / T, batch), dim3(256), 0, s, src, src_stride, dst, dst_stride, S,
-                       static_cast<const MfmaFoldPlan*>(plans), w2, partials, T);
+    const bool pub = flagged && mle_multifold2_partials(S) == kFlagRecsPerTable && (S >> (2 * kMfmaMaxJ)) >= 16u;
+    const MfmaFoldPlan* pl = static_cast<const MfmaFoldPlan*>(plans);
+    if (pub)
+        hipExtLaunchKernelGGL(k_mle_multifold2_mfma<true>, dim3((S >> 8) / T, batch), dim3(256), 0, s, nullptr, ended, 0, src, src_stride, dst, dst_stride, S, pl,
+                              w2, partials, T, flagged, flag_ticket);
+    else
+        hipLaunchKernelGGL(k_mle_multifold2_mfma<false>, dim3((S >> 8) / T, batch), dim3(256), 0, s, src, src_stride, dst, dst_stride, S, pl, w2, partials, T,
+                           (uint64_t*)nullptr, 0u);
+    return pub;
 }
 
 void launch_mle_round_reduce(const MlePartial* partials, uint32_t nblk, uint32_t batch, MleHostRec* host_rec,
diff --git a/gkr_amd/csrc/options.h b/gkr_amd/csrc/options.h
--- a/gkr_amd/csrc/options.h
+++ b/gkr_amd/csrc/options.h
@@ -11,6 +11,7 @@
     X(first_fold_levels, "first_fold_levels", "GKR_FIRST_FOLD_LEVELS", 0, "variables the first fold of a host-hashed 2^18 .. 2^24-point sumcheck binds: 1 five, 2 ten in the one read (0: the default, capi_internal.h kMleFirstFoldLevels)") \
     X(pass0_stream, "pass0_stream", "GKR_PASS0_STREAM", 0, "pass 0 of a streaming launch of the plain sumcheck: 1 k_mle_sub_sums (a block per partial), 2 its pipelined form (a wave per one or two partials, 16-byte loads kept in flight in two sets) where it applies, 3 as 2 with the rolling form (a wave per partial, ONE buffer of sixteen loads, every XCD on a contiguous eighth of the launch) in place of the form of two partials per wave (0: the default, kernels.h kMlePass0Stream)") \
     X(fold2_tiles, "fold2_tiles", "GKR_FOLD2_TILES", 0, "64-entry tiles a block of the two-level first fold takes: k forces min(k, 2^(n-16)), a power of two (0: one, which is fastest where measured)") \
+    X(stream_publish, "stream_publish", "GKR_STREAM_PUBLISH", 0, "streaming passes of a batch in several groups on the two-level schedule (the rolling pass 0, the two-level first fold; not the call's last streaming launch): 1 every pass publishes through k_mle_sub_reduce, 2 their blocks publish flag-in-word records to pinned memory, which the hashing threads total -- no reduce launch between two streaming launches (0: the default, 2)") \
     X(no_fused_reduce, "no_fused_reduce", "GKR_NO_FUSED_REDUCE", 0, "latency-bound passes publish through k_mle_sub_reduce instead of from their last block") \
     X(hash_chunk, "hash_chunk", "GKR_HASH_CHUNK", 0, "8 or 16: sumchecks per host hash call (0: 16 when host threads are scarce)")    \
     X(device_hash_percent, "device_hash_percent", "GKR_DEVICE_HASH_PERCENT", 0, "share of a batch of >= 64 plain sumchecks hashed on the device (0..90)") \
```

New measurement: 512.2 billion (median of 6 runs). 2.1% higher.
